# seung-lab/crackle

Hardware: AMD Instinct MI355X
Metric: voxels/s encode+decode, 1024x1024x512 uint32; bit-exact .ckl bytes (higher is better)
Workload: dtype u32

## Files before the change

crackle_amd/csrc/ckl_encode.hip:

```cpp
#include "ckl_encoder.hpp"
#include "ckl_decoder.hpp"
#include "ckl_runs.hpp"
#include "ckl_strips.hpp"
#include "ckl_trail.hpp"
#include "ckl_recompress.hpp"
#include "ckl_erode.hpp"

#include <algorithm>
#include <atomic>
#include <chrono>
#include <functional>
#include <memory>
#include <mutex>

namespace ckl {

using namespace dev;

template <typename LABEL>
__global__ void __launch_bounds__(kBlock) k_stats(const LABEL* __restrict__ labels, uint64_t voxels, unsigned long long* __restrict__ out ) {
	__shared__ unsigned long long s_max[kWaves], s_pairs[kWaves];
	unsigned long long mx = 0, pairs = 0;
	const uint64_t stride = static_cast<uint64_t>(gridDim.x) * kBlock;
	for (uint64_t i = static_cast<uint64_t>(blockIdx.x) * kBlock + threadIdx.x; i < voxels; i += stride) {
// ... 667 lines not shown
	const dim3 grid(static_cast<uint32_t>((threads + kBlock - 1) / kBlock), static_cast<uint32_t>(sz));
	if (four) hipLaunchKernelGGL(k_paint_components4, grid, dim3(kBlock), 0, s, planeV, row_words, plane_words, static_cast<uint32_t>(sx), sxy, word_base, rbase, run_cc, comp_off, id_base, out);
	else hipLaunchKernelGGL(k_paint_components, grid, dim3(kBlock), 0, s, planeV, row_words, plane_words, static_cast<uint32_t>(sx), sxy, word_base, rbase, run_cc, comp_off, id_base, out);
}

__global__ void __launch_bounds__(kBlock) k_bitonic_step(uint64_t* __restrict__ a, uint32_t j, uint32_t k, uint32_t n) {
	const uint32_t i = blockIdx.x * kBlock + threadIdx.x;
	if (i >= n) return;
	const uint32_t l = i ^ j;
	if (l > i) {
		const uint64_t x = a[i], y = a[l];
		const bool up = (i & k) == 0;
		if ((x > y) == up) { a[i] = y; a[l] = x; }
	}
}
__global__ void __launch_bounds__(kBlock) k_bitonic_step2(uint64_t* __restrict__ a, uint32_t j, uint32_t k, uint32_t n) {
	const uint32_t t = blockIdx.x * kBlock + threadIdx.x;
	if (t >= n / 4u) return;
	const uint32_t h = j >> 1;
	const uint32_t lb = static_cast<uint32_t>(__ffs(h)) - 1u;
	const uint32_t i = (t & (h - 1u)) | ((t >> lb) << (lb + 2u));
	uint64_t v0 = a[i], v1 = a[i | h], v2 = a[i | j], v3 = a[i | j | h];
	const bool up = (i & k) == 0;
	auto cx = [&](uint64_t& x, uint64_t& y) { if ((x > y) == up) { const uint64_t z = x; x = y; y = z; } };
	cx(v0, v2); cx(v1, v3);
	cx(v0, v1); cx(v2, v3);
	a[i] = v0; a[i | h] = v1; a[i | j] = v2; a[i | j | h] = v3;
}

__global__ void __launch_bounds__(kBlock) k_bitonic_first(uint64_t* __restrict__ a, uint32_t n) {
	__shared__ uint64_t s[2048];
	const uint32_t base = blockIdx.x * 2048u;
	for (uint32_t t = threadIdx.x; t < 2048u; t += kBlock) s[t] = base + t < n ? a[base + t] : ~0ull;
	__syncthreads();
	for (uint32_t k = 2; k <= 2048u; k <<= 1) {
		for (uint32_t j = k >> 1; j > 0; j >>= 1) {
			for (uint32_t t = threadIdx.x; t < 2048u; t += kBlock) {
				const uint32_t l = t ^ j;
				if (l > t) {
					const uint64_t x = s[t], y = s[l];
					const bool up = ((base + t) & k) == 0;
					if ((x > y) == up) { s[t] = y; s[l] = x; }
				}
			}
			__syncthreads();
		}
	}
	for (uint32_t t = threadIdx.x; t < 2048u; t += kBlock) if (base + t < n) a[base + t] = s[t];
}
__global__ void __launch_bounds__(kBlock) k_bitonic_local(uint64_t* __restrict__ a, uint32_t j_start, uint32_t k, uint32_t n) {
	__shared__ uint64_t s[2048];
	const uint32_t base = blockIdx.x * 2048u;
	for (uint32_t t = threadIdx.x; t < 2048u; t += kBlock) s[t] = base + t < n ? a[base + t] : ~0ull;
	__syncthreads();
	for (uint32_t j = j_start; j > 0; j >>= 1) {
		for (uint32_t t = threadIdx.x; t < 2048u; t += kBlock) {
			const uint32_t l = t ^ j;
			if (l > t) {
				const uint64_t x = s[t], y = s[l];
				const bool up = ((base + t) & k) == 0;
				if ((x > y) == up) { s[t] = y; s[l] = x; }
			}
		}
		__syncthreads();
	}
	for (uint32_t t = threadIdx.x; t < 2048u; t += kBlock) if (base + t < n) a[base + t] = s[t];
}
__global__ void __launch_bounds__(kBlock) k_pad_copy_u64(const uint64_t* __restrict__ src, uint64_t n, uint64_t* __restrict__ dst, uint64_t n_pad) {
	const uint64_t i = static_cast<uint64_t>(blockIdx.x) * kBlock + threadIdx.x;
	if (i < n_pad) dst[i] = i < n ? src[i] : ~0ull;
}
constexpr uint32_t kUniqPer = 8, kUniqItems = kBlock * kUniqPer;
__device__ __forceinline__ uint32_t unique_heads(const uint64_t* __restrict__ sorted, uint32_t n, uint32_t i0, uint64_t (&v)[kUniqPer]) {
	uint32_t flag = 0;
#pragma unroll
	for (uint32_t q = 0; q < kUniqPer; q++) {
		const uint32_t i = i0 + q;
		v[q] = i < n ? sorted[i] : 0;
		const uint64_t prev = q ? v[q - 1] : ((i > 0 && i < n) ? sorted[i - 1] : 0);
		flag |= ((i < n && (i == 0 || v[q] != prev)) ? 1u : 0u) << q;
	}
	return flag;
}
__global__ void __launch_bounds__(kBlock) k_unique_count(const uint64_t* __restrict__ sorted, uint32_t n, uint32_t* __restrict__ blk_count) {
	__shared__ uint32_t s_red[kWaves];
	uint64_t v[kUniqPer];
	const uint32_t flag = unique_heads(sorted, n, blockIdx.x * kUniqItems + threadIdx.x * kUniqPer, v);
	const uint32_t tot = block_sum(static_cast<uint32_t>(__popc(flag)), s_red);
	if (threadIdx.x == 0) blk_count[blockIdx.x] = tot;
}
__global__ void __launch_bounds__(kBlock) k_unique_scan(uint32_t* __restrict__ blk_count, uint32_t nblk, uint32_t* __restrict__ n_uniq) {
	__shared__ uint32_t s_scan[kWaves];
	uint32_t carry = 0;
	for (uint32_t b0 = 0; b0 < nblk; b0 += kBlock) {
		const uint32_t b = b0 + threadIdx.x;
		uint32_t c[1] = { b < nblk ? blk_count[b] : 0u }, tot[1];
		block_excl_add<1>(c, tot, s_scan);
		if (b < nblk) blk_count[b] = carry + c[0];
		carry += tot[0];
	}
	if (threadIdx.x == 0) *n_uniq = carry;
}
__global__ void __launch_bounds__(kBlock) k_unique_scatter(const uint64_t* __restrict__ sorted, uint32_t n, const uint32_t* __restrict__ blk_base, uint64_t* __restrict__ uniq) {
	__shared__ uint32_t s_scan[kWaves];
	uint64_t v[kUniqPer];
	const uint32_t flag = unique_heads(sorted, n, blockIdx.x * kUniqItems + threadIdx.x * kUniqPer, v);
	uint32_t c[1] = { static_cast<uint32_t>(__popc(flag)) }, tot[1];
	block_excl_add<1>(c, tot, s_scan);
	uint32_t o = blk_base[blockIdx.x] + c[0];
#pragma unroll
	for (uint32_t q = 0; q < kUniqPer; q++) if ((flag >> q) & 1u) uniq[o++] = v[q];
}

constexpr uint64_t kLabelHashEmpty = ~0ull;
__device__ __forceinline__ uint32_t label_hash(uint64_t v) {
	v ^= v >> 33; v *= 0xff51afd7ed558ccdull; v ^= v >> 33;
	return static_cast<uint32_t>(v);
}
__global__ void __launch_bounds__(kBlock) k_label_hash_insert(const uint64_t* __restrict__ mapping, uint32_t n, unsigned long long* __restrict__ table, uint32_t mask, uint32_t* __restrict__ has_max) {
	const uint32_t i = blockIdx.x * kBlock + threadIdx.x;
	if (i >= n) return;
	const unsigned long long v = mapping[i];
	if (v == kLabelHashEmpty) { *has_max = 1u; return; }
	uint32_t h = label_hash(v) & mask;
	for (uint32_t probe = 0; probe <= mask; probe++) {
		const unsigned long long seen = table[h];
		if (seen == v) return;
		if (seen == kLabelHashEmpty) {
			const unsigned long long old = atomicCAS(table + h, kLabelHashEmpty, v);
			if (old == kLabelHashEmpty || old == v) return;
		}
		h = (h + 1u) & mask;
	}
}
__device__ __forceinline__ uint32_t hash_occupied(const unsigned long long* __restrict__ table, uint32_t slots, uint32_t i0, uint64_t (&v)[kUniqPer]) {
	uint32_t flag = 0;
#pragma unroll
	for (uint32_t q = 0; q < kUniqPer; q++) {
		v[q] = i0 + q < slots ? table[i0 + q] : kLabelHashEmpty;
		flag |= (v[q] != kLabelHashEmpty ? 1u : 0u) << q;
	}
	return flag;
}
__global__ void __launch_bounds__(kBlock) k_label_hash_count(const unsigned long long* __restrict__ table, uint32_t slots, uint32_t* __restrict__ blk_count) {
	__shared__ uint32_t s_red[kWaves];
	uint64_t v[kUniqPer];
	const uint32_t flag = hash_occupied(table, slots, blockIdx.x * kUniqItems + threadIdx.x * kUniqPer, v);
	const uint32_t tot = block_sum(static_cast<uint32_t>(__popc(flag)), s_red);
	if (threadIdx.x == 0) blk_count[blockIdx.x] = tot;
}
__global__ void __launch_bounds__(kBlock) k_label_hash_scatter(
	const unsigned long long* __restrict__ table, uint32_t slots, const uint32_t* __restrict__ blk_base, const uint32_t* __restrict__ n_found,
	const uint32_t* __restrict__ has_max, uint64_t* __restrict__ out
) {
	__shared__ uint32_t s_scan[kWaves];
	uint64_t v[kUniqPer];
	const uint32_t flag = hash_occupied(table, slots, blockIdx.x * kUniqItems + threadIdx.x * kUniqPer, v);
	uint32_t c[1] = { static_cast<uint32_t>(__popc(flag)) }, tot[1];
	block_excl_add<1>(c, tot, s_scan);
	uint32_t o = blk_base[blockIdx.x] + c[0];
#pragma unroll
	for (uint32_t q = 0; q < kUniqPer; q++) if ((flag >> q) & 1u) out[o++] = v[q];
	if (blockIdx.x == 0 && threadIdx.x == 0 && *has_max) out[*n_found] = kLabelHashEmpty;
}

__global__ void __launch_bounds__(kBlock) k_flat_section(
	const uint64_t* __restrict__ uniq, const uint32_t* __restrict__ n_uniq, int stored_width,
	const uint32_t* __restrict__ ncomp, uint32_t nslices, int component_width,
	const uint64_t* __restrict__ mapping, uint32_t n, uint8_t* __restrict__ out, uint32_t* __restrict__ missing
) {
	const uint32_t nu = *n_uniq;
	const int key_width = nu <= 0xFFu ? 1 : (nu <= 0xFFFFu ? 2 : 4);
	const uint32_t i = blockIdx.x * kBlock + threadIdx.x;
	if (i == 0) for (int b = 0; b < 8; b++) out[b] = static_cast<uint8_t>((static_cast<uint64_t>(nu) >> (8 * b)) & 0xFF);
	uint8_t* o_uniq = out + 8;
	uint8_t* o_cc = o_uniq + static_cast<uint64_t>(nu) * stored_width;
	uint8_t* o_keys = o_cc + static_cast<uint64_t>(nslices) * component_width;
	if (i < nu) {
		const uint64_t v = uniq[i];
		for (int b = 0; b < stored_width; b++) o_uniq[static_cast<uint64_t>(i) * stored_width + b] = static_cast<uint8_t>((v >> (8 * b)) & 0xFF);
	}
	if (i < nslices) {
		const uint32_t v = ncomp[i];
		for (int b = 0; b < component_width; b++) o_cc[static_cast<uint64_t>(i) * component_width + b] = b < 4 ? static_cast<uint8_t>((v >> (8 * b)) & 0xFF) : 0;
	}
	if (i < n) {
		const uint64_t v = mapping[i];
		uint32_t lo = 0, hi = nu;
		while (lo + 1 < hi) {
			const uint32_t mid = (lo + hi) >> 1;
			if (uniq[mid] <= v) lo = mid; else hi = mid;
		}
		if (missing && (nu == 0 || uniq[lo] != v)) *missing = 1u;
		for (int b = 0; b < key_width; b++) o_keys[static_cast<uint64_t>(i) * key_width + b] = static_cast<uint8_t>((lo >> (8 * b)) & 0xFF);
	}
}

__global__ void __launch_bounds__(kBlock) k_code_offsets(
	const uint32_t* __restrict__ boc_len, const uint32_t* __restrict__ payload_len, const uint32_t* __restrict__ slice_err,
	uint32_t nslices, uint64_t* __restrict__ out_off, uint32_t* __restrict__ report
) {
	__shared__ unsigned long long s_part[kBlock];
	__shared__ uint32_t s_err;
	if (threadIdx.x == 0) s_err = 0;
	const uint32_t per = (nslices + kBlock - 1) / kBlock;
	const uint32_t z0 = threadIdx.x * per, z1 = min(z0 + per, nslices);
	unsigned long long sum = 0;
	uint32_t err = 0;
	for (uint32_t z = z0; z < z1; z++) { sum += static_cast<unsigned long long>(boc_len[z]) + payload_len[z]; err |= slice_err[z]; }
	s_part[threadIdx.x] = sum;
	__syncthreads();
	if (err) atomicOr(&s_err, err);
	if (threadIdx.x == 0) {
		unsigned long long run = 0;
		for (uint32_t i = 0; i < kBlock; i++) { const unsigned long long v = s_part[i]; s_part[i] = run; run += v; }
		report[nslices] = static_cast<uint32_t>(run); report[nslices + 1] = static_cast<uint32_t>(run >> 32);
	}
	__syncthreads();
	unsigned long long off = s_part[threadIdx.x];
	for (uint32_t z = z0; z < z1; z++) {
		const uint32_t len = boc_len[z] + payload_len[z];
		out_off[z] = off;
		report[z] = len;
		off += len;
	}
	if (threadIdx.x == 0) report[nslices + 2] = s_err;
}

__global__ void __launch_bounds__(kBlock) k_gather_codes(
	const uint8_t* __restrict__ boc, const uint64_t* __restrict__ bbase, const uint32_t* __restrict__ boc_len,
	const uint8_t* __restrict__ payload, const uint64_t* __restrict__ pbase, const uint32_t* __restrict__ payload_len,
	const uint64_t* __restrict__ out_off, uint8_t* __restrict__ out
) {
	const uint32_t zi = blockIdx.x;
	uint8_t* o = out + out_off[zi];
	const uint32_t nb = boc_len[zi], np = payload_len[zi];
	const uint8_t* b = boc + bbase[zi];
	const uint8_t* p = payload + pbase[zi];
	for (uint32_t i = threadIdx.x; i < nb; i += kBlock) o[i] = b[i];
	for (uint32_t i = threadIdx.x; i < np; i += kBlock) o[nb + i] = p[i];
}

struct CrcShifts { uint32_t x[8]; };
__global__ void __launch_bounds__(kBlock) k_crc32c_pieces(const uint8_t* __restrict__ data, uint64_t n, uint64_t pad, uint32_t P, CrcShifts sh, uint32_t* __restrict__ parts) {
	__shared__ uint32_t s_tab[256];
	__shared__ uint32_t s_st[kBlock];
	{
		uint32_t c = threadIdx.x;
		for (int k = 0; k < 8; k++) c = (c & 1u) ? (c >> 1) ^ dev::kCrcPoly : (c >> 1);
		s_tab[threadIdx.x] = c;
	}
	__syncthreads();
	const uint64_t f0 = (static_cast<uint64_t>(blockIdx.x) * kBlock + threadIdx.x) * P;
	uint32_t c = 0;
	for (uint32_t g = 0; g < P; g += 16) {
		const int64_t m0 = static_cast<int64_t>(f0 + g) - static_cast<int64_t>(pad);
		uint32_t w[4] = { 0, 0, 0, 0 };
		if (m0 >= 0 && static_cast<uint64_t>(m0) + 16u <= n) __builtin_memcpy(w, data + m0, 16);
		else if (m0 + 16 > 0) for (int b = 0; b < 16; b++) { const int64_t i = m0 + b; if (i >= 0 && static_cast<uint64_t>(i) < n) w[b >> 2] |= static_cast<uint32_t>(data[i]) << (8 * (b & 3)); }
#pragma unroll
		for (int b = 0; b < 16; b++) c = s_tab[(c ^ (w[b >> 2] >> (8 * (b & 3)))) & 0xFFu] ^ (c >> 8);
	}
	s_st[threadIdx.x] = c;
	__syncthreads();
	for (int k = 0; k < 8; k++) {
		const uint32_t stride = 1u << k;
		if ((threadIdx.x & (2u * stride - 1u)) == 0u) s_st[threadIdx.x] = gf_mul(s_st[threadIdx.x], sh.x[k]) ^ s_st[threadIdx.x + stride];
		__syncthreads();
	}
	if (threadIdx.x == 0) parts[blockIdx.x] = s_st[0];
}
__global__ void __launch_bounds__(kBlock) k_crc32c_fold(const uint32_t* __restrict__ parts, uint32_t G, CrcShifts sh, uint32_t init_term, uint32_t* __restrict__ out) {
	__shared__ uint32_t s_st[kBlock];
	s_st[threadIdx.x] = threadIdx.x < G ? parts[threadIdx.x] : 0u;
	__syncthreads();
	for (int k = 0; (1u << k) < G; k++) {
		const uint32_t stride = 1u << k;
		if ((threadIdx.x & (2u * stride - 1u)) == 0u && threadIdx.x + stride < G) s_st[threadIdx.x] = gf_mul(s_st[threadIdx.x], sh.x[k]) ^ s_st[threadIdx.x + stride];
		__syncthreads();
	}
	if (threadIdx.x == 0) out[0] = ~(s_st[0] ^ init_term);
}

__global__ void __launch_bounds__(kBlock) k_copy_bytes(const uint8_t* __restrict__ src, uint8_t* __restrict__ dst, uint64_t n) {
	const uint64_t head = min(n, static_cast<uint64_t>((4u - (reinterpret_cast<uintptr_t>(dst) & 3u)) & 3u));
	const uint64_t words = (n - head) / 4u;
	const uint64_t tid = static_cast<uint64_t>(blockIdx.x) * kBlock + threadIdx.x;
	const uint64_t stride = static_cast<uint64_t>(gridDim.x) * kBlock;
	if (tid < head) dst[tid] = src[tid];
	const uint64_t tail0 = head + words * 4u;
	if (tid < n - tail0) dst[tail0 + tid] = src[tail0 + tid];
	const uint8_t* s0 = src + head;
	const uint32_t sh = static_cast<uint32_t>(reinterpret_cast<uintptr_t>(s0) & 3u) * 8u;
	const uint32_t* sw = reinterpret_cast<const uint32_t*>(reinterpret_cast<uintptr_t>(s0) & ~static_cast<uintptr_t>(3));
	uint32_t* dw = reinterpret_cast<uint32_t*>(dst + head);
	if (sh == 0u) {
		for (uint64_t i = tid; i < words; i += stride) dw[i] = sw[i];
	}
	else {
		for (uint64_t i = tid; i < words; i += stride) dw[i] = __funnelshift_r(sw[i], sw[i + 1], sh);
	}
}

__global__ void __launch_bounds__(kBlock) k_trail_step_kinds(const uint32_t* __restrict__ events, const uint64_t* __restrict__ ibase, const uint32_t* __restrict__ n_events, uint32_t* __restrict__ counts) {
	__shared__ uint32_t s_c[5];
	const uint32_t zi = blockIdx.x;
	if (threadIdx.x < 5) s_c[threadIdx.x] = 0u;
	__syncthreads();
	const uint32_t n = n_events[zi] & ~(dev::kEvFormatAddr12 | dev::kEvWalkWide);
	const uint32_t* ev = events + ibase[zi];
	uint32_t c[4] = { 0, 0, 0, 0 };
	for (uint32_t i = threadIdx.x; i < n; i += kBlock) c[ev[i] >> 30]++;
	for (int k = 0; k < 4; k++) if (c[k]) atomicAdd(&s_c[k], c[k]);
	if (threadIdx.x == 0) {
		uint32_t run = 0, longest = 0;
		for (uint32_t i = 0; i < n; i++) { if ((ev[i] >> 30) == 1u) run = 0; else { run++; longest = run > longest ? run : longest; } }
		s_c[4] = longest;
	}
	__syncthreads();
	if (threadIdx.x < 5) counts[zi * 5u + threadIdx.x] = s_c[threadIdx.x];
}

}

using namespace ckl;

static void crc32c_device(const uint8_t* data, uint64_t n, uint32_t* parts, uint32_t* out, hipStream_t s) {
	uint32_t P = 128, G = 1;
	while (G < static_cast<uint32_t>(kBlock) && static_cast<uint64_t>(G) * kBlock * P < n) G <<= 1;
	if (static_cast<uint64_t>(G) * kBlock * P < n) P = static_cast<uint32_t>(((n + static_cast<uint64_t>(G) * kBlock - 1) / (static_cast<uint64_t>(G) * kBlock) + 15) / 16 * 16);
	const uint64_t frame = static_cast<uint64_t>(G) * kBlock * P;
	static std::mutex shifts_mutex;
	static uint32_t shifts_for = 0;
	static CrcShifts shifts_in, shifts_over;
	CrcShifts in_wg, over_wg;
	{
		std::lock_guard<std::mutex> lock(shifts_mutex);
		if (shifts_for != P) {
			for (int k = 0; k < 8; k++) {
				shifts_in.x[k] = gf_xpow(8ull * P << k);
				shifts_over.x[k] = gf_xpow(8ull * P * kBlock << k);
			}
			shifts_for = P;
		}
		in_wg = shifts_in; over_wg = shifts_over;
	}
	hipLaunchKernelGGL(k_crc32c_pieces, dim3(G), dim3(kBlock), 0, s, data, n, frame - n, P, in_wg, parts);
	hipLaunchKernelGGL(k_crc32c_fold, dim3(1), dim3(kBlock), 0, s, parts, G, over_wg, gf_mul(0xFFFFFFFFu, gf_xpow(8ull * n)), out);
}

static void copy_bytes_device(const uint8_t* src, uint8_t* dst, uint64_t n, hipStream_t s) {
	if (!n) return;
	const uint32_t blocks = static_cast<uint32_t>(std::min<uint64_t>((n / 4u + kBlock - 1) / kBlock + 1u, 8192u));
	hipLaunchKernelGGL(k_copy_bytes, dim3(blocks), dim3(kBlock), 0, s, src, dst, n);
}

namespace {

struct UploadPacker {
	struct Item { void* buf; size_t off, count; void (*bind)(void*, uint8_t*, size_t); };
	std::vector<Item> items;
	std::vector<uint8_t> image;
	template <typename T>
	void add(DevBuf<T>& dst, const std::vector<T>& src) {
		const size_t off = (image.size() + 255) & ~static_cast<size_t>(255);
		image.resize(off + std::max<size_t>(src.size(), 1) * sizeof(T));
		if (!src.empty()) memcpy(image.data() + off, src.data(), src.size() * sizeof(T));
		items.push_back({ &dst, off, src.size(), [](void* b, uint8_t* base, size_t n) { static_cast<DevBuf<T>*>(b)->borrow(reinterpret_cast<T*>(base), n); } });
	}
	void commit(DevBuf<uint8_t>& block, hipStream_t s, void** staging = nullptr) {
		if (image.empty()) return;
		for (const Item& it : items) it.bind(it.buf, nullptr, 0);
		block.ensure(image.size());
		if (staging) {
			if (*staging) host_out_free(*staging);
			*staging = host_out_alloc(std::max<size_t>(image.size(), 64u << 10));
			memcpy(*staging, image.data(), image.size());
			upload_small(block.p, *staging, image.size(), s, *staging);
		}
		else CKL_HIP(hipMemcpyAsync(block.p, image.data(), image.size(), hipMemcpyHostToDevice, s));
		for (const Item& it : items) it.bind(it.buf, block.p + it.off, it.count);
	}
};

template <typename LABEL>
VolumeStats volume_stats(ckl_encoder& e, const LABEL* labels, uint64_t voxels) {
	VolumeStats st;
	if (voxels == 0) return st;
	hipStream_t s = e.stream;
	e.d_stats.ensure(2);
	CKL_HIP(hipMemsetAsync(e.d_stats.p, 0, 2 * sizeof(unsigned long long), s));
	const uint32_t blocks = static_cast<uint32_t>(std::min<uint64_t>((voxels + kBlock - 1) / kBlock, 256ull * 8));
	hipLaunchKernelGGL(k_stats<LABEL>, dim3(blocks), dim3(kBlock), 0, s, labels, voxels, e.d_stats.p);
	auto r = download(e.d_stats.p, 2, s);
	st.max_label = r[0]; st.pairs = r[1];
	LABEL f, l;
	CKL_HIP(hipMemcpy(&f, labels, sizeof(LABEL), hipMemcpyDeviceToHost));
	CKL_HIP(hipMemcpy(&l, labels + (voxels - 1), sizeof(LABEL), hipMemcpyDeviceToHost));
	st.first = f; st.last = l;
	return st;
}

inline uint32_t* plane_v(const ckl_encoder& e) { return e.d_planes.p; }
inline uint32_t* plane_h(const ckl_encoder& e, uint32_t ns) { return e.d_planes.p + e.plane_words * ns; }

inline bool planes_cached(const ckl_encoder& e, const void* labels, int64_t sx, int64_t sy, int64_t sz) {
	return e.planes_for == labels && e.planes_dims[0] == sx && e.planes_dims[1] == sy && e.planes_dims[2] == sz;
}

inline uint64_t crack_edges(const ckl_encoder& e, int64_t sx, int64_t sy, size_t zi, bool permissible) {
	const uint64_t interior = static_cast<uint64_t>(sx > 0 ? sx - 1 : 0) * sy + static_cast<uint64_t>(sx) * (sy > 0 ? sy - 1 : 0);
	const uint64_t differ = static_cast<uint64_t>(e.count_v[zi]) + e.count_h[zi];
	return permissible ? interior - differ : differ;
}

void planes_collect(ckl_encoder& e, uint32_t ns, VolumeStats* st, const std::vector<unsigned long long>* fetched = nullptr) {
	std::vector<unsigned long long> mine;
	if (!fetched) { mine = download(e.d_plane_out.p, 4ull * ns, e.stream); fetched = &mine; }
	const std::vector<unsigned long long>& o = *fetched;
	e.count_v.resize(ns); e.count_h.resize(ns);
	VolumeStats v;
	for (uint32_t zi = 0; zi < ns; zi++) {
		e.count_v[zi] = static_cast<uint32_t>(o[4ull * zi]);
		e.count_h[zi] = static_cast<uint32_t>(o[4ull * zi + 1]);
		v.pairs += o[4ull * zi + 2];
		v.max_label = std::max<uint64_t>(v.max_label, o[4ull * zi + 3]);
	}
	e.planes_deferred = false;
	if (st) *st = v;
}

void trail_prezero(ckl_encoder& e, int64_t sx, int64_t sy, int64_t sz) {
	hipStream_t s = e.stream2;
	const uint32_t ns = static_cast<uint32_t>(sz);
	const uint64_t nverts = static_cast<uint64_t>(sx + 1) * (sy + 1);
	const uint32_t start_words = static_cast<uint32_t>((nverts + 31) / 32);
	e.d_slice_err.ensure(ns);
	e.t_counters.ensure(7 * static_cast<size_t>(ns));
	e.t_start_bits.ensure(static_cast<size_t>(start_words) * ns);
	CKL_HIP(hipMemsetAsync(e.d_slice_err.p, 0, ns * sizeof(uint32_t), s));
	CKL_HIP(hipMemsetAsync(e.t_counters.p, 0, 7 * static_cast<size_t>(ns) * sizeof(uint32_t), s));
	CKL_HIP(hipMemsetAsync(e.t_start_bits.p, 0, static_cast<size_t>(start_words) * ns * sizeof(uint32_t), s));
	CKL_HIP(hipEventRecord(e.ev_prezero, s));
	e.trail_zeroed = true;
}

template <typename LABEL>
void planes_pass(ckl_encoder& e, const LABEL* labels, int64_t sx, int64_t sy, int64_t sz, VolumeStats* st, bool defer = false) {
	hipStream_t s = e.stream;
	const uint32_t ns = static_cast<uint32_t>(sz);
	e.trail_zeroed = false;
	e.planes_deferred = false;
	e.row_words = static_cast<uint32_t>((sx + 31) / 32);
	e.plane_words = static_cast<uint64_t>(e.row_words) * sy;
	e.d_planes.ensure(2 * e.plane_words * ns);
	constexpr uint32_t P = 16 / sizeof(LABEL);
	const bool fast = !getenv("CKL_PLANES_GENERIC") && sx >= static_cast<int64_t>(P) && sx % P == 0 && (reinterpret_cast<uintptr_t>(labels) & 15u) == 0;
	if (fast) {
		const uint32_t strips = static_cast<uint32_t>((sx + 64 * P - 1) / (64 * P));
		const uint32_t bands = static_cast<uint32_t>((sy + kBandRows - 1) / kBandRows);
		const uint32_t nblk = (strips * bands + kWaves - 1) / kWaves;
		e.d_plane_partial.ensure(4ull * nblk * ns);
		e.d_plane_partial_max.ensure(static_cast<size_t>(nblk) * ns);
		e.d_plane_out.ensure(4ull * ns + 1);
		trail_prezero(e, sx, sy, sz);
		hipLaunchKernelGGL(k_label_planes_stream<LABEL>, dim3(nblk, ns), dim3(kBlock), 0, s,
			labels, static_cast<uint32_t>(sx), static_cast<uint32_t>(sy), strips, bands,
			plane_v(e), plane_h(e, ns), e.row_words, e.plane_words,
			e.d_plane_partial.p, e.d_plane_partial_max.p, e.d_plane_out.p + 4ull * ns);
		hipLaunchKernelGGL(k_planes_reduce, dim3(ns), dim3(kBlock), 0, s, e.d_plane_partial.p, e.d_plane_partial_max.p, nblk, e.d_plane_out.p, e.d_plane_out.p + 4ull * ns);
		e.planes_deferred = defer;
		if (!e.planes_deferred) planes_collect(e, ns, st);
		return;
	}
	if (st) *st = volume_stats<LABEL>(e, labels, static_cast<uint64_t>(sx) * sy * sz);
	e.d_count_vh.ensure(2 * static_cast<size_t>(ns));
	CKL_HIP(hipMemsetAsync(e.d_count_vh.p, 0, 2 * static_cast<size_t>(ns) * sizeof(uint32_t), s));
	const uint32_t chunks = static_cast<uint32_t>((sx + 63) / 64);
	const uint64_t units = static_cast<uint64_t>(chunks) * sy;
	hipLaunchKernelGGL(k_label_planes<LABEL>, dim3(static_cast<uint32_t>((units + kWaves * kPlaneUnroll - 1) / (kWaves * kPlaneUnroll)), ns), dim3(kBlock), 0, s,
		labels, static_cast<uint32_t>(sx), static_cast<uint32_t>(sy), chunks,
		plane_v(e), plane_h(e, ns), e.row_words, e.plane_words,
		e.d_count_vh.p, e.d_count_vh.p + ns);
	std::vector<uint32_t> c = download(e.d_count_vh.p, 2 * static_cast<size_t>(ns), s);
	e.count_v.assign(c.begin(), c.begin() + ns);
	e.count_h.assign(c.begin() + ns, c.end());
}

void planes_pass_any(ckl_encoder& e, const void* labels, int64_t sx, int64_t sy, int64_t sz, VolumeStats* st) {
	with_label_type(e.dtype_bytes, [&](auto t) { planes_pass(e, static_cast<const typename decltype(t)::type*>(labels), sx, sy, sz, st); });
}

enum class GraphFormat : uint32_t { IMPERMISSIBLE = 0, PERMISSIBLE = 1, ON_DEVICE = 2 };
inline GraphFormat graph_format(bool permissible) { return permissible ? GraphFormat::PERMISSIBLE : GraphFormat::IMPERMISSIBLE; }
void graph_pass(ckl_encoder& e, int64_t sx, int64_t sy, int64_t sz, GraphFormat format, VolumeStats* st = nullptr) {
	hipStream_t s = e.stream;
	const uint32_t ns = static_cast<uint32_t>(sz);
	e.tiles_x = static_cast<uint32_t>((sx + 1 + kTrailTileDim - 1) / kTrailTileDim);
	e.tiles_y = static_cast<uint32_t>((sy + 1 + 7) / 8);
	const uint32_t mtx = static_cast<uint32_t>((sx + 1 + 7) / 8), mty = static_cast<uint32_t>((sy + 1 + 7) / 8);
	e.mtx2 = (mtx + 1) / 2;
	e.adjm_stride = static_cast<uint64_t>(e.mtx2) * ((mty + 1) / 2) * 4 * 2;
	e.d_adjm.ensure(e.adjm_stride * ns);
	e.graph_blocks = (e.tiles_x * e.tiles_y + kBlock - 1) / kBlock;
	e.t_blk_special.ensure(static_cast<size_t>(e.graph_blocks) * ns);
	e.t_blk_corner.ensure(static_cast<size_t>(e.graph_blocks) * ns);
	e.d_count_vh.ensure(4 * static_cast<size_t>(ns));
	const bool on_device = format == GraphFormat::ON_DEVICE;
	if (on_device && !e.planes_deferred) throw Error(CKL_ERR_RUNTIME, "crackle_amd: internal: crack format left to the device without deferred counts");
	const unsigned long long half_voxels = static_cast<unsigned long long>(static_cast<int64_t>(static_cast<uint64_t>(sx) * sy * sz) / 2);
	hipLaunchKernelGGL(k_trail_graph, dim3(e.graph_blocks, ns), dim3(kBlock), 0, s,
		plane_v(e), plane_h(e, ns), e.row_words, e.plane_words,
		static_cast<uint32_t>(sx), static_cast<uint32_t>(sy), static_cast<uint32_t>(format),
		on_device ? e.d_plane_out.p + 4ull * ns : nullptr, half_voxels,
		reinterpret_cast<uint32_t*>(e.d_adjm.p), e.adjm_stride * 4,
		e.mtx2, e.tiles_x, e.tiles_y, e.t_blk_special.p, e.t_blk_corner.p);
	hipLaunchKernelGGL(k_trail_count_scan, dim3(ns), dim3(kBlock), 0, s, e.t_blk_special.p, e.t_blk_corner.p, e.graph_blocks,
		e.d_count_vh.p + 2 * static_cast<size_t>(ns), e.d_count_vh.p + 3 * static_cast<size_t>(ns));
	std::vector<unsigned long long> po;
	if (e.planes_deferred) {
		po.resize(4ull * ns);
		CKL_HIP(hipMemcpyAsync(po.data(), e.d_plane_out.p, po.size() * sizeof(unsigned long long), hipMemcpyDeviceToHost, s));
	}
	std::vector<uint32_t> c = download(e.d_count_vh.p + 2 * static_cast<size_t>(ns), 2 * static_cast<size_t>(ns), s);
	e.count_special.assign(c.begin(), c.begin() + ns);
	e.count_corner.assign(c.begin() + ns, c.end());
	VolumeStats v;
	if (!po.empty()) planes_collect(e, ns, &v, &po);
	if (st && !po.empty()) *st = v;
	e.graph_permissible = on_device ? static_cast<int64_t>(v.pairs) < static_cast<int64_t>(static_cast<uint64_t>(sx) * sy * sz) / 2 : format == GraphFormat::PERMISSIBLE;
}

enum class CrackGoal { HISTOGRAM, CODES };
struct CrackRequest {
	CrackGoal goal = CrackGoal::CODES;
	bool permissible = false;
	int markov_order = 0;
	const std::vector<uint8_t>* model = nullptr;
	bool reuse_trail = false;
	std::function<void()> overlap;
};
struct CrackResult {
	std::vector<uint32_t> code_len;
	uint64_t total = 0;
	bool any_chain = false;
	std::vector<uint32_t> hist;
	std::vector<uint8_t> model;
};

inline size_t trail_walk_lds(uint32_t max_special) { return (static_cast<size_t>(max_special) + 256) * 16 + 1024; }

FinishArgs finish_args(const ckl_encoder& e, int64_t sx, int64_t sy, int markov_order) {
	FinishArgs fa;
	fa.sx = static_cast<int>(sx); fa.sy = static_cast<int>(sy);
	fa.xw = byte_width(static_cast<uint64_t>(sx) + 1); fa.yw = byte_width(static_cast<uint64_t>(sy) + 1);
	fa.markov = markov_order ? 1u : 0u;
	fa.cbase = e.d_cbase.p; fa.kbase = e.d_kbase.p;
	fa.n_chains = e.d_n_chains.p; fa.n_raw = e.d_n_raw.p; fa.n_valid = e.d_n_valid.p;
	fa.cp = e.d_cp.p; fa.chain_node = e.d_chain_node.p; fa.chain_off = e.d_chain_off.p; fa.chain_clen = e.d_chain_clen.p;
	fa.chain_order = e.d_chain_order.p; fa.chain_dst = e.d_chain_dst.p; fa.chain_vstart = e.d_chain_vstart.p;
	fa.fcode = e.d_fcode.p; fa.dcode = e.d_dcode.p;
	fa.pbase = e.d_pbase.p; fa.payload = e.d_payload.p; fa.bbase = e.d_bbase.p; fa.boc = e.d_boc.p;
	fa.payload_len = e.d_payload_len.p; fa.boc_len = e.d_boc_len.p;
	fa.z0 = 0;
	return fa;
}

TrailArgs trail_args(const ckl_encoder& e, int64_t sx, int64_t sy, uint32_t ns) {
	const uint64_t nverts = static_cast<uint64_t>(sx + 1) * (sy + 1);
	TrailArgs ta;
	ta.adjm = e.d_adjm.p; ta.adjm_stride = e.adjm_stride; ta.mtx2 = e.mtx2; ta.tiles_x = e.tiles_x; ta.tiles_y = e.tiles_y;
	ta.planeV = plane_v(e); ta.planeH = plane_h(e, ns); ta.row_words = e.row_words; ta.plane_words = e.plane_words;
	ta.sx = static_cast<uint32_t>(sx); ta.sy = static_cast<uint32_t>(sy); ta.inv = e.graph_permissible ? 0xFFFFFFFFu : 0u;
	ta.sxe = static_cast<uint32_t>(sx + 1); ta.sye = static_cast<uint32_t>(sy + 1); ta.nverts = static_cast<uint32_t>(nverts);
	ta.max_steps = e.t_max_steps.p;
	ta.nbase = e.t_nbase.p; ta.ncap = e.t_ncap.p;
	ta.n_nodes = e.t_counters.p; ta.n_corners = e.t_counters.p + 2 * ns;
	ta.n_starts = e.t_counters.p + 3 * ns; ta.n_items = e.t_counters.p + 4 * ns;
	ta.node_vertex = e.t_node_vertex.p; ta.node_adj = e.t_node_adj.p; ta.vert2node = e.t_vert2node.p;
	ta.cobase = e.t_cobase.p; ta.cocap = e.t_cocap.p; ta.corner_vertex = e.t_corner_vertex.p;
	ta.dart_end = e.t_dart_end.p; ta.dart_len = e.t_dart_len.p; ta.dart_minv = e.t_dart_minv.p; ta.dart_minpos = e.t_dart_minpos.p;
	ta.dart_codes = e.t_dart_codes.p; ta.dart_inline = e.t_dart_inline.p;
	ta.parent = e.t_parent.p; ta.compmin = e.t_compmin.p;
	ta.start_bits = e.t_start_bits.p; ta.start_words = static_cast<uint32_t>((nverts + 31) / 32); ta.starts = e.t_starts.p;
	ta.ibase = e.t_ibase.p; ta.icap = e.t_icap.p; ta.items = e.t_items.p; ta.item_off = e.t_item_off.p;
	ta.sbase = e.d_sbase.p; ta.scap = e.d_scap.p; ta.stack_node = e.d_stack_node.p; ta.stack_item = e.d_stack_code.p;
	ta.kbase = e.d_kbase.p; ta.kcap = e.d_kcap.p;
	ta.chain_node = e.d_chain_node.p; ta.chain_item0 = e.t_chain_item0.p; ta.chain_off = e.d_chain_off.p; ta.chain_clen = e.d_chain_clen.p;
	ta.n_chains = e.d_n_chains.p; ta.n_raw = e.d_n_raw.p; ta.n_valid = e.d_n_valid.p;
	ta.cbase = e.d_cbase.p; ta.ccap = e.d_ccap.p; ta.cp = e.d_cp.p; ta.slice_err = e.d_slice_err.p;
	ta.events = e.t_events.p; ta.n_events = e.t_counters.p + 5 * ns; ta.seg_len_sum = e.t_counters.p + 6 * ns; ta.chain_ev0 = e.t_chain_ev0.p; ta.ev_lnd = e.t_ev_lnd.p; ta.ev_item = e.t_ev_item.p;
	ta.dbg = nullptr;
	{ const char* env = getenv("CKL_TRAIL_WALK"); ta.walk_plain = (env && !strcmp(env, "plain")) ? 1u : 0u; ta.walk_no_regs = (env && !strcmp(env, "lds")) ? 1u : 0u; }
	{ const char* env = getenv("CKL_TRAIL_WALK_STACK"); ta.walk_stack_cap = env ? static_cast<uint32_t>(std::max(1, atoi(env))) : 0xFFFFFFFFu; }
	ta.graph_blocks = e.graph_blocks; ta.blk_special = e.t_blk_special.p; ta.blk_corner = e.t_blk_corner.p;
	ta.z0 = 0;
	return ta;
}

void trail_diag(ckl_encoder& e, uint32_t ns, const unsigned long long* ta_dbg, uint32_t max_special, size_t trail_lds_used) {
	hipStream_t s = e.stream;
	std::vector<uint32_t> c = download(e.t_counters.p, 5 * static_cast<size_t>(ns), s);
	double m[5] = { 0 };
	for (int k = 0; k < 5; k++) for (uint32_t zi = 0; zi < ns; zi++) m[k] += static_cast<double>(c[static_cast<size_t>(k) * ns + zi]) / ns;
	double sp = 0, co = 0;
	for (uint32_t zi = 0; zi < ns; zi++) { sp += static_cast<double>(e.count_special[zi]) / ns; co += static_cast<double>(e.count_corner[zi]) / ns; }
	if (ta_dbg) {
		std::vector<unsigned long long> g = download(ta_dbg, 16, s);
		if (g[11]) fprintf(stderr, "[ckl trail diag, k_trail_walk] mean cycles per slice: table fill=%.0f fill + walk=%.0f\n", static_cast<double>(g[6]) / g[11], static_cast<double>(g[7]) / g[11]);
		if (g[11]) fprintf(stderr, "[ckl trail diag, k_trail_walk] slices=%llu iterations/slice=%.0f cycles/iteration=%.0f clock=%.2f GHz (cycles / 100 MHz ticks)\n",
			g[11], static_cast<double>(g[8]) / g[11], g[8] ? static_cast<double>(g[9]) / g[8] : 0.0, g[10] ? static_cast<double>(g[9]) / (g[10] * 10.0) : 0.0);
		fprintf(stderr, "[ckl trail diag, k_trail_components, mean cycles per slice] union=%.0f component minima=%.0f starts/splits=%.0f bitmap scan=%.0f\n",
			static_cast<double>(g[12]) / ns, static_cast<double>(g[13]) / ns, static_cast<double>(g[14]) / ns, static_cast<double>(g[15]) / ns);
		fprintf(stderr, "[ckl trail diag, k_trail_segments] waves=%llu iterations/wave mean=%.1f max=%llu cycles/wave mean=%.0f max=%llu cycles/iteration=%.0f active lanes/iteration=%.1f\n",
			g[4], g[4] ? static_cast<double>(g[0]) / g[4] : 0.0, g[1], g[4] ? static_cast<double>(g[2]) / g[4] : 0.0, g[3],
			g[0] ? static_cast<double>(g[2]) / g[0] : 0.0, g[0] ? static_cast<double>(g[5]) / g[0] : 0.0);
	}
	fprintf(stderr, "[ckl trail diag] max degree-1/3/4 vertices of a slice=%u, k_trail_walk LDS=%zu bytes\n", max_special, trail_lds_used);
	fprintf(stderr, "[ckl trail diag, mean per slice] degree-1/3/4 vertices=%.0f corners=%.0f nodes=%.0f starts=%.0f items=%.0f\n", sp, co, m[0], m[3], m[4]);
}

void check_walk_errors(ckl_encoder& e, uint32_t ns) {
	const std::vector<uint32_t> errs = download(e.d_slice_err.p, ns, e.stream);
	for (uint32_t zi = 0; zi < ns; zi++) if (errs[zi]) throw Error(CKL_ERR_RUNTIME, "crackle_amd: crack walk scratch overflow on z=" + std::to_string(zi));
}

CrackResult crack_pass(ckl_encoder& e, int64_t sx, int64_t sy, int64_t sz, const CrackRequest& rq) {
	hipStream_t s = e.stream;
	const uint32_t ns = static_cast<uint32_t>(sz);
	const uint64_t nverts = static_cast<uint64_t>(sx + 1) * (sy + 1);
	const int markov_order = rq.markov_order;
	const bool reuse_trail = rq.reuse_trail;
	if (rq.goal == CrackGoal::HISTOGRAM && (!markov_order || rq.model)) throw Error(CKL_ERR_RUNTIME, "crackle_amd: internal: a markov histogram needs an order and no model");
	CrackResult result;
	e.d_slice_err.ensure(ns);
	const bool prezeroed = e.trail_zeroed && !reuse_trail;
	e.trail_zeroed = false;
	if (prezeroed) CKL_HIP(hipStreamWaitEvent(s, e.ev_prezero, 0));
	if (!reuse_trail && !prezeroed) CKL_HIP(hipMemsetAsync(e.d_slice_err.p, 0, ns * sizeof(uint32_t), s));

	std::vector<uint64_t> cbase(ns), sbase(ns), kbase(ns);
	std::vector<uint32_t> ccap(ns), scap(ns), kcap(ns), max_steps(ns);
	std::vector<uint64_t> nbase(ns), cobase(ns), ibase(ns);
	std::vector<uint32_t> ncap(ns), cocap(ns), icap(ns);
	uint64_t ctot = 0, stot = 0, ktot = 0, ntot = 0, cotot = 0, itot = 0;
	uint32_t max_ncap = 0, max_cocap = 0, max_icap = 0, max_special = 0;
	bool any = false;
	for (uint32_t zi = 0; zi < ns; zi++) {
		const uint64_t E = crack_edges(e, sx, sy, zi, rq.permissible);
		any = any || E > 0;
		const uint64_t cc = ((7 * E + 16 + 15) / 16) * 16;
		if (cc > 0xFFFFFFF0ull) throw Error(CKL_ERR_RUNTIME, "crackle_amd: slice has too many crack edges");
		cbase[zi] = ctot; ccap[zi] = static_cast<uint32_t>(cc); ctot += cc;
		max_steps[zi] = static_cast<uint32_t>(E + 1);
		const uint64_t nc = ((static_cast<uint64_t>(e.count_special[zi]) + e.count_corner[zi] + 16) / 16) * 16;
		if (nc >= (1ull << 28)) throw Error(CKL_ERR_RUNTIME, "crackle_amd: slice has too many crack vertices");
		nbase[zi] = ntot; ncap[zi] = static_cast<uint32_t>(nc); ntot += nc;
		cobase[zi] = cotot; cocap[zi] = e.count_corner[zi]; cotot += e.count_corner[zi];
		const uint64_t ic = 7 * nc + 16;
		ibase[zi] = itot; icap[zi] = static_cast<uint32_t>(ic); itot += ic;
		sbase[zi] = stot; scap[zi] = static_cast<uint32_t>(2 * nc + 4); stot += 2 * nc + 4;
		kbase[zi] = ktot; kcap[zi] = static_cast<uint32_t>(nc); ktot += nc;
		max_ncap = std::max<uint32_t>(max_ncap, ncap[zi]);
		max_cocap = std::max<uint32_t>(max_cocap, cocap[zi]);
		max_icap = std::max<uint32_t>(max_icap, icap[zi]);
		max_special = std::max<uint32_t>(max_special, e.count_special[zi]);
	}
	result.any_chain = any;
	if (g_ht && g_ht->on) {
		uint32_t over = 0;
		for (uint32_t zi = 0; zi < ns; zi++) over += e.count_special[zi] > 3584u;
		fprintf(stderr, "[ckl trail nodes] max special %u, slices above 3584: %u of %u\n", max_special, over, ns);
	}
	HT_MARK("c:caps");

	UploadPacker tables;
	tables.add(e.d_cbase, cbase); tables.add(e.d_ccap, ccap);
	tables.add(e.d_sbase, sbase); tables.add(e.d_scap, scap);
	tables.add(e.d_kbase, kbase); tables.add(e.d_kcap, kcap);
	e.d_cp.ensure(ctot); e.d_fcode.ensure(ctot);
	if (markov_order) e.d_dcode.ensure(ctot);
	e.d_stack_node.ensure(stot); e.d_stack_code.ensure(stot);
	e.d_chain_node.ensure(ktot); e.d_chain_off.ensure(ktot); e.d_chain_clen.ensure(ktot);
	e.d_chain_order.ensure(ktot); e.d_chain_dst.ensure(ktot); e.d_chain_vstart.ensure(ktot);
	e.d_n_chains.ensure(ns); e.d_n_raw.ensure(ns); e.d_n_valid.ensure(ns);
	e.d_payload_len.ensure(ns); e.d_boc_len.ensure(ns);
	const int xw = byte_width(static_cast<uint64_t>(sx) + 1), yw = byte_width(static_cast<uint64_t>(sy) + 1);
	std::vector<uint64_t> pbase(ns), bbase(ns);
	uint64_t ptot = 0, btot = 0;
	for (uint32_t zi = 0; zi < ns; zi++) {
		const uint64_t ncodes = ccap[zi];
		const uint64_t pbytes = markov_order ? (3ull * ncodes + 2 + 7) / 8 : (ncodes + 3) / 4;
		pbase[zi] = ptot; ptot += ((pbytes + 8 + 3) / 4) * 4;
		const uint64_t bbytes = 4 + yw + static_cast<uint64_t>(kcap[zi]) * (yw + 2 * xw);
		bbase[zi] = btot; btot += bbytes;
	}
	tables.add(e.d_pbase, pbase); tables.add(e.d_bbase, bbase);
	tables.add(e.t_nbase, nbase); tables.add(e.t_ncap, ncap);
	tables.add(e.t_cobase, cobase); tables.add(e.t_cocap, cocap);
	tables.add(e.t_ibase, ibase); tables.add(e.t_icap, icap);
	tables.add(e.t_max_steps, max_steps);
	tables.commit(e.d_crack_tables, s, e.uploads_by_kernel ? &e.tables_staging : nullptr);
	HT_MARK("c:tables");
	e.d_payload.ensure(ptot + 8); e.d_boc.ensure(btot + 8);
	e.codes_capacity = ptot + btot;
	if (markov_order) CKL_HIP(hipMemsetAsync(e.d_payload.p, 0, ptot + 8, s));

	DevBuf<unsigned long long> d_tdbg;
	size_t trail_lds_used = 0;
	if (!reuse_trail) {
		e.t_counters.ensure(7 * static_cast<size_t>(ns));
		if (!prezeroed) CKL_HIP(hipMemsetAsync(e.t_counters.p, 0, 7 * static_cast<size_t>(ns) * sizeof(uint32_t), s));
		e.t_node_vertex.ensure(ntot); e.t_node_adj.ensure(ntot + 16); e.t_vert2node.ensure(nverts * ns);
		e.t_corner_vertex.ensure(cotot);
		e.t_dart_end.ensure(4 * ntot); e.t_dart_len.ensure(4 * ntot); e.t_dart_minv.ensure(4 * ntot); e.t_dart_minpos.ensure(4 * ntot);
		e.t_dart_codes.ensure(4 * ntot); e.t_dart_inline.ensure(4 * ntot);
		e.t_parent.ensure(ntot); e.t_compmin.ensure(ntot); e.t_starts.ensure(ntot);
		const uint32_t start_words = static_cast<uint32_t>((nverts + 31) / 32);
		e.t_start_bits.ensure(static_cast<size_t>(start_words) * ns);
		if (!prezeroed) CKL_HIP(hipMemsetAsync(e.t_start_bits.p, 0, static_cast<size_t>(start_words) * ns * sizeof(uint32_t), s));
		e.t_items.ensure(itot); e.t_item_off.ensure(itot); e.t_chain_item0.ensure(ktot);
		e.t_events.ensure(itot); e.t_chain_ev0.ensure(ktot); e.t_ev_lnd.ensure(itot); e.t_ev_item.ensure(itot);
		e.last_trail_slices = ns;

		TrailArgs ta = trail_args(e, sx, sy, ns);
		const FinishArgs fa = finish_args(e, sx, sy, markov_order);
		if (kTuning && getenv("CKL_TRAIL_DIAG")) { d_tdbg.ensure(16); CKL_HIP(hipMemsetAsync(d_tdbg.p, 0, 128, s)); ta.dbg = d_tdbg.p; }
		int max_lds = 0;
		CKL_HIP(hipDeviceGetAttribute(&max_lds, hipDeviceAttributeMaxSharedMemoryPerBlock, e.device));
		const size_t budget = static_cast<size_t>(max_lds > 1024 ? max_lds - 1024 : 0);
		const uint32_t dart_blocks = (4 * max_ncap + kWalkChunk * kWaves - 1) / (kWalkChunk * kWaves);
		size_t clds = (static_cast<size_t>(max_special) + 1024) * 12;
		if (const char* env = getenv("CKL_TRAIL_LDS")) clds = static_cast<size_t>(std::max(0, atoi(env)));
		clds = (std::min(budget, std::max<size_t>(clds, 1024)) / 16) * 16;
		CKL_HIP(hipFuncSetAttribute(reinterpret_cast<const void*>(&k_trail_components), hipFuncAttributeMaxDynamicSharedMemorySize, static_cast<int>(clds)));
		size_t lds = trail_walk_lds(max_special);
		if (const char* env = getenv("CKL_TRAIL_LDS")) lds = static_cast<size_t>(std::max(0, atoi(env)));
		lds = std::min(budget, std::max<size_t>(lds, 4096));
		lds = (lds / 16) * 16;
		CKL_HIP(hipFuncSetAttribute(reinterpret_cast<const void*>(&k_trail_walk), hipFuncAttributeMaxDynamicSharedMemorySize, static_cast<int>(lds)));
		trail_lds_used = lds;
		HT_MARK("c:setup");

		if (any) {
			hipLaunchKernelGGL(k_trail_nodes, dim3(e.graph_blocks, ns), dim3(kBlock), 0, s, ta);
			hipLaunchKernelGGL(k_trail_segments, dim3(dart_blocks, ns), dim3(kBlock), 0, s, ta);
			if (max_cocap) hipLaunchKernelGGL(k_trail_loops, dim3((max_cocap + kBlock - 1) / kBlock, ns), dim3(kBlock), 0, s, ta);
			hipLaunchKernelGGL(k_trail_components, dim3(ns), dim3(kCompBlock), clds, s, ta, static_cast<uint32_t>(clds));
		}
		CKL_HIP(hipEventRecord(e.evd0, s));
		hipLaunchKernelGGL(k_trail_walk, dim3(ns), dim3(kWave), lds, s, ta, static_cast<uint32_t>(lds));
		CKL_HIP(hipEventRecord(e.evd1, s));
		hipLaunchKernelGGL(k_trail_items, dim3(ns), dim3(kItemsBlock), 0, s, ta);
		hipLaunchKernelGGL(k_trail_offsets, dim3(ns), dim3(kBlock), 0, s, ta);
		hipLaunchKernelGGL(k_trail_expand, dim3((max_icap + kExpandChunk * kWaves - 1) / (kExpandChunk * kWaves), ns), dim3(kBlock), 0, s, ta);
		hipLaunchKernelGGL(k_finish, dim3(ns), dim3(kFinishBlock), 0, s, fa);
	}
	HT_MARK("c:enqueue");
	if (kTuning && getenv("CKL_TRAIL_DIAG")) trail_diag(e, ns, d_tdbg.p, max_special, trail_lds_used);

	auto enqueue_tail = [&]() {
		e.d_out_off.ensure(ns);
		e.d_code_report.ensure(static_cast<size_t>(ns) + 3);
		e.d_codes_out.ensure(e.codes_capacity + 8);
		hipLaunchKernelGGL(k_code_offsets, dim3(1), dim3(kBlock), 0, s, e.d_boc_len.p, e.d_payload_len.p, e.d_slice_err.p, ns, e.d_out_off.p, e.d_code_report.p);
		hipLaunchKernelGGL(k_gather_codes, dim3(ns), dim3(kBlock), 0, s, e.d_boc.p, e.d_bbase.p, e.d_boc_len.p,
			e.d_payload.p, e.d_pbase.p, e.d_payload_len.p, e.d_out_off.p, e.d_codes_out.p);
	};
	if (!markov_order) enqueue_tail();
	if (rq.overlap) rq.overlap();
	HT_MARK("c:overlap");

	if (markov_order) {
		if (rq.model) result.model = *rq.model;
		else {
			const size_t rows = static_cast<size_t>(1) << (2 * markov_order);
			e.d_hist.ensure(rows * 4);
			CKL_HIP(hipMemsetAsync(e.d_hist.p, 0, rows * 4 * sizeof(uint32_t), s));
			const uint32_t hist_lds = (rows * 4 <= 16384) ? static_cast<uint32_t>(rows * 4) : 0u;
			if (hist_lds * 4 > 48 * 1024) CKL_HIP(hipFuncSetAttribute(reinterpret_cast<const void*>(&k_markov_hist), hipFuncAttributeMaxDynamicSharedMemorySize, static_cast<int>(hist_lds * 4)));
			hipLaunchKernelGGL(k_markov_hist, dim3(ns), dim3(kBlock), hist_lds * sizeof(uint32_t), s, e.d_dcode.p, e.d_cbase.p, e.d_n_valid.p, markov_order, e.d_hist.p, hist_lds);
			result.hist = download(e.d_hist.p, rows * 4, s);
			if (rq.goal == CrackGoal::HISTOGRAM) { check_walk_errors(e, ns); return result; }
			result.model = markov_stats_to_model(result.hist.data(), rows);
		}
		upload(e.d_model, result.model, s);
		hipLaunchKernelGGL(k_markov_pack, dim3(ns), dim3(kBlock), 0, s, e.d_dcode.p, e.d_cbase.p, e.d_n_valid.p, markov_order,
			e.d_model.p, e.d_pbase.p, e.d_payload.p, e.d_payload_len.p);
		enqueue_tail();
	}
	HT_MARK("c:finish_enq");
	const std::vector<uint32_t> report = download(e.d_code_report.p, static_cast<size_t>(ns) + 3, s);
	HT_MARK("c:finish_wait");
	if (report[ns + 2]) check_walk_errors(e, ns);
	result.code_len.assign(report.begin(), report.begin() + ns);
	result.total = static_cast<uint64_t>(report[ns]) | (static_cast<uint64_t>(report[ns + 1]) << 32);
	return result;
}

struct FlatResult {
	std::vector<uint32_t> ncomp;
	std::vector<uint32_t> crcs;
	uint64_t total = 0;
};

void ensure_geom_table(ckl_encoder& e, uint64_t sxy) {
	if (e.g_table_pixels == sxy && e.d_G.p) return;
	hipStream_t s = e.stream2;
	const uint32_t npx = static_cast<uint32_t>(sxy);
	const uint32_t B = 1024, nblk = npx / B + 1;
	std::vector<uint32_t> g_base(B), blk_g(nblk), blk_x(nblk);
	const uint32_t X = gf_xpow(32);
	g_base[0] = 0;
	for (uint32_t i = 1; i < B; i++) g_base[i] = gf_mul(X, g_base[i - 1] ^ 0x80000000u);
	const uint32_t gB = gf_mul(X, g_base[B - 1] ^ 0x80000000u);
	const uint32_t XB = gf_xpow(32ull * B);
	blk_g[0] = 0; blk_x[0] = 0x80000000u;
	for (uint32_t k = 1; k < nblk; k++) {
		blk_g[k] = blk_g[k - 1] ^ gf_mul(blk_x[k - 1], gB);
		blk_x[k] = gf_mul(blk_x[k - 1], XB);
	}
	DevBuf<uint32_t> t_base, t_g, t_x;
	upload(t_base, g_base, s); upload(t_g, blk_g, s); upload(t_x, blk_x, s);
	e.d_G.ensure(static_cast<size_t>(npx) + 1);
	hipLaunchKernelGGL(k_build_geom_table, dim3(npx / kBlock + 1), dim3(kBlock), 0, s, t_base.p, t_g.p, t_x.p, npx, e.d_G.p);
	CKL_HIP(hipStreamSynchronize(s));
	e.g_table_pixels = sxy;
}

RunArrays flat_arrays(const ckl_encoder& e) {
	RunArrays ra;
	ra.word_base = e.d_word_base.p; ra.rbase = e.d_rbase.p; ra.rcap = e.d_rcap.p;
	ra.parent = e.d_parent.p; ra.run_start = e.d_run_start.p; ra.run_cc = e.d_run_cc.p;
	ra.nruns = e.d_nruns.p; ra.ncomp = e.d_ncomp.p; ra.slice_err = e.d_slice_err2.p;
	ra.comp_pix = e.d_comp_pix.p;
	return ra;
}

void flat_report_layout(ckl_encoder& e, uint32_t ns, hipStream_t s) {
	e.d_flat_report.ensure(4 * static_cast<size_t>(ns) + 1);
	e.d_ncomp.borrow(e.d_flat_report.p, ns); e.d_crc_acc.borrow(e.d_flat_report.p + ns, ns);
	e.d_idbits.borrow(e.d_flat_report.p + 2 * static_cast<size_t>(ns), ns); e.d_slice_err2.borrow(e.d_flat_report.p + 3 * static_cast<size_t>(ns), ns);
	CKL_HIP(hipMemsetAsync(e.d_slice_err2.p, 0, (static_cast<size_t>(ns) + 1) * sizeof(uint32_t), s));
}

RunGeom flat_geom(const ckl_encoder& e, int64_t sx, int64_t sy, uint32_t ns) {
	RunGeom g;
	g.planeV = plane_v(e); g.planeH = plane_h(e, ns);
	g.row_words = e.row_words; g.plane_words = e.plane_words;
	g.flip = 1u;
	g.sx = static_cast<uint32_t>(sx); g.sy = static_cast<uint32_t>(sy);
	return g;
}

void flat_enqueue_runs(ckl_encoder& e, int64_t sx, int64_t sy, int64_t sz) {
	hipStream_t s = e.stream2;
	const uint32_t ns = static_cast<uint32_t>(sz);
	const uint64_t sxy = static_cast<uint64_t>(sx) * sy;
	e.flat_strips = false;

	std::vector<uint64_t>& rbase = e.h_rbase;
	std::vector<uint32_t>& rcap = e.h_rcap;
	rbase.assign(ns, 0); rcap.assign(ns, 0);
	uint64_t rtot = 0;
	uint32_t max_rcap = 0;
	for (uint32_t zi = 0; zi < ns; zi++) {
		const uint64_t runs = static_cast<uint64_t>(sy) + e.count_v[zi];
		rbase[zi] = rtot; rcap[zi] = static_cast<uint32_t>(runs); rtot += runs;
		max_rcap = std::max<uint32_t>(max_rcap, static_cast<uint32_t>(runs));
	}
	upload(e.d_rbase, rbase, s); upload(e.d_rcap, rcap, s);
	e.d_word_base.ensure(e.plane_words * ns);
	e.d_parent.ensure(rtot); e.d_run_start.ensure(rtot); e.d_run_cc.ensure(rtot); e.d_comp_pix.ensure(rtot);
	e.d_nruns.ensure(ns);
	flat_report_layout(e, ns, s);

	const RunGeom g = flat_geom(e, sx, sy, ns);
	const RunArrays ra = flat_arrays(e);
	hipLaunchKernelGGL(k_run_index, dim3(ns), dim3(kIndexBlock), 0, s, g, ra);
	launch_run_union(s, ns, g, ra);
	ResolveScratch rs;
	rs.nblk = (max_rcap + kBlock - 1) / kBlock;
	e.d_run_local.ensure(rtot);
	e.d_blk_roots.ensure(static_cast<size_t>(rs.nblk) * ns);
	rs.run_local = e.d_run_local.p; rs.blk_roots = e.d_blk_roots.p;
	launch_run_resolve(s, ns, ra, rs, e.d_G.p, static_cast<uint32_t>(sxy), 0u, e.d_crc_acc.p, e.d_idbits.p);
	HT_MARK("f:enqueue_runs");
}

uint32_t flat_resolve_cap(size_t lds_bytes) {
	uint32_t cap = static_cast<uint32_t>(std::min<size_t>(kResolveCap, (lds_bytes - (kMaxStrips + 64u) * 4u) / 4u));
	if (const char* env = getenv("CKL_ENC_RESOLVE_CAP")) cap = std::min<uint32_t>(cap, static_cast<uint32_t>(std::max(1, atoi(env))));
	return cap;
}
uint32_t flat_resolve_cap_max(ckl_encoder& e) {
	if (!e.max_lds) CKL_HIP(hipDeviceGetAttribute(&e.max_lds, hipDeviceAttributeMaxSharedMemoryPerBlock, e.device));
	return flat_resolve_cap(static_cast<size_t>(e.max_lds) - 8192u);
}

bool flat_strip_plan(ckl_encoder& e, int64_t sx, int64_t sy, uint32_t ns) {
	if (getenv("CKL_ENC_LABEL_RUNS")) return false;
	const uint64_t sxy = static_cast<uint64_t>(sx) * sy;
	if (e.row_words == 0 || e.row_words > kStripWords || sxy >= 0xFFFF0000ull) return false;
	uint64_t runs_max = 0, comps_min = 0;
	const uint64_t pairs_up = static_cast<uint64_t>(sx) * (sy - 1);
	for (uint32_t zi = 0; zi < ns; zi++) {
		const uint64_t runs = static_cast<uint64_t>(sy) + e.count_v[zi];
		const uint64_t equal_up = pairs_up - std::min<uint64_t>(pairs_up, e.count_h[zi]);
		runs_max = std::max<uint64_t>(runs_max, runs);
		comps_min = std::max<uint64_t>(comps_min, runs > equal_up ? runs - equal_up : 0ull);
	}
	const double runs_per_row = static_cast<double>(runs_max) / static_cast<double>(sy);
	const uint32_t fit = static_cast<uint32_t>(0.7 * kEncStripCap / runs_per_row);
	if (fit < 1u) return false;
	const uint32_t rows = std::max<uint32_t>(1u, std::min<uint32_t>(kStripWords / e.row_words, fit));
	const uint32_t nstrips = (static_cast<uint32_t>(sy) + rows - 1) / rows;
	if (nstrips > kMaxStrips || comps_min > flat_resolve_cap_max(e)) return false;
	e.flat_strip_rows = rows; e.flat_nstrips = nstrips;
	e.flat_strip_cap = static_cast<uint32_t>(std::min<uint64_t>(kEncStripCap, static_cast<uint64_t>(rows) * sx));
	if (const char* env = getenv("CKL_ENC_STRIP_CAP")) e.flat_strip_cap = std::min<uint32_t>(e.flat_strip_cap, static_cast<uint32_t>(std::max(1, atoi(env))));
	return true;
}

StripArrays flat_strip_arrays(const ckl_encoder& e) {
	StripArrays sa = {};
	sa.run_lid = e.s_run_lid.p; sa.sc_w = e.s_sc_w.p; sa.sc_cc = e.s_sc_first.p;
	sa.strip_nruns = e.s_strip_nruns.p; sa.strip_nsc = e.s_strip_nsc.p;
	sa.seam_first = e.s_seam_first.p; sa.seam_last = e.s_seam_last.p;
	sa.slice_err = e.d_slice_err2.p; sa.overflow = e.d_flat_report.p + 4 * e.d_ncomp.n;
	sa.nstrips = e.flat_nstrips; sa.strip_rows = e.flat_strip_rows; sa.cap = e.flat_strip_cap; sa.zbase = 0;
	return sa;
}

void flat_launch_resolve(ckl_encoder& e, const void* labels, int64_t sx, int64_t sy, uint32_t ns, uint32_t cap) {
	hipStream_t s = e.stream2;
	e.flat_resolve_cap = cap;
	e.d_label_slots.ensure(static_cast<size_t>(ns) * cap);
	ResolveArgs ra = {};
	ra.cap = cap;
	EncResolve en;
	en.labels = labels; en.sxy = static_cast<uint64_t>(sx) * sy; en.slots = e.d_label_slots.p; en.crc_acc = e.d_crc_acc.p; en.idbits = e.d_idbits.p;
	const RunGeom g = flat_geom(e, sx, sy, ns);
	const StripArrays sa = flat_strip_arrays(e);
	const size_t tab_bytes = static_cast<size_t>(cap) * sizeof(uint32_t);
	if (e.label_src) {
		if (tab_bytes > 48u * 1024u) CKL_HIP(hipFuncSetAttribute(reinterpret_cast<const void*>(&k_slice_resolve_enc_pixels), hipFuncAttributeMaxDynamicSharedMemorySize, static_cast<int>(tab_bytes)));
		hipLaunchKernelGGL(k_slice_resolve_enc_pixels, dim3(ns), dim3(kResolveBlock), tab_bytes, s, g, sa, ra, en, e.d_ncomp.p);
		return;
	}
	with_label_type(e.dtype_bytes, [&](auto t) {
		typedef typename decltype(t)::type LABEL;
		if (tab_bytes > 48u * 1024u) CKL_HIP(hipFuncSetAttribute(reinterpret_cast<const void*>(&k_slice_resolve_enc<LABEL>), hipFuncAttributeMaxDynamicSharedMemorySize, static_cast<int>(tab_bytes)));
		hipLaunchKernelGGL(k_slice_resolve_enc<LABEL>, dim3(ns), dim3(kResolveBlock), tab_bytes, s, g, sa, ra, en, e.d_ncomp.p);
	});
}

void flat_enqueue(ckl_encoder& e, const void* labels, int64_t sx, int64_t sy, int64_t sz, bool need_runs, bool beside_walk) {
	hipStream_t s = e.stream2;
	const uint32_t ns = static_cast<uint32_t>(sz);
	const uint64_t sxy = static_cast<uint64_t>(sx) * sy;
	ensure_geom_table(e, sxy);
	if (need_runs || !beside_walk || !flat_strip_plan(e, sx, sy, ns)) { flat_enqueue_runs(e, sx, sy, sz); return; }
	e.flat_strips = true;
	const size_t nst = static_cast<size_t>(e.flat_nstrips) * ns;
	e.s_strip_nruns.ensure(nst); e.s_strip_nsc.ensure(nst);
	e.s_seam_first.ensure(nst * e.row_words); e.s_seam_last.ensure(nst * e.row_words);
	e.s_run_lid.ensure(nst * e.flat_strip_cap); e.s_sc_w.ensure(nst * e.flat_strip_cap); e.s_sc_first.ensure(nst * e.flat_strip_cap);
	flat_report_layout(e, ns, s);
	hipLaunchKernelGGL(k_strip_ccl_enc, dim3(e.flat_nstrips, ns), dim3(kBlock), 0, s, flat_geom(e, sx, sy, ns), flat_strip_arrays(e), e.d_G.p, static_cast<uint32_t>(sxy));
	flat_launch_resolve(e, labels, sx, sy, ns, flat_resolve_cap(kFlatResolveLds));
	HT_MARK("f:enqueue_strips");
}

template <typename LABEL>
void flat_collect(ckl_encoder& e, const LABEL* labels, int64_t sx, int64_t sy, int64_t sz, FlatResult& out) {
	hipStream_t s = e.stream2;
	const uint32_t ns = static_cast<uint32_t>(sz);
	const uint64_t sxy = static_cast<uint64_t>(sx) * sy;
	const size_t rep_n = 4 * static_cast<size_t>(ns) + 1;
	std::vector<uint32_t> rep = download(e.d_flat_report.p, rep_n, s);
	if (e.flat_strips && rep[rep_n - 1] == 2u && e.flat_resolve_cap < flat_resolve_cap_max(e)) {
		CKL_HIP(hipMemsetAsync(e.d_flat_report.p + rep_n - 1, 0, sizeof(uint32_t), s));
		flat_launch_resolve(e, labels, sx, sy, ns, flat_resolve_cap_max(e));
		HT_MARK("f:resolve_retry");
		rep = download(e.d_flat_report.p, rep_n, s);
	}
	if (e.flat_strips && rep[rep_n - 1]) {
		flat_enqueue_runs(e, sx, sy, sz);
		rep = download(e.d_flat_report.p, rep_n, s);
	}
	const uint32_t *acc = rep.data() + ns, *idbits = rep.data() + 2 * static_cast<size_t>(ns), *errs = rep.data() + 3 * static_cast<size_t>(ns);
	out.ncomp.assign(rep.begin(), rep.begin() + ns);
	HT_MARK(e.flat_strips ? "f:wait_strips" : "f:wait_runs");
	for (uint32_t zi = 0; zi < ns; zi++) if (errs[zi]) throw Error(CKL_ERR_RUNTIME, "crackle_amd: run table overflow on z=" + std::to_string(zi));
	const uint32_t init_term = gf_mul(0xFFFFFFFFu, gf_xpow(32ull * sxy));
	out.crcs.resize(ns);
	uint32_t fix_bits = 0xFFFFFFFFu, fix = 0;
	for (uint32_t zi = 0; zi < ns; zi++) {
		if (idbits[zi] != fix_bits) { fix_bits = idbits[zi]; fix = gf_xpow(32 - fix_bits); }
		out.crcs[zi] = ~(gf_mul(acc[zi], fix) ^ init_term);
	}

	std::vector<uint64_t>& comp_off = e.h_comp_off;
	comp_off.assign(ns, 0);
	uint64_t total = 0;
	for (uint32_t zi = 0; zi < ns; zi++) { comp_off[zi] = total; total += out.ncomp[zi]; }
	upload(e.d_comp_off, comp_off, s);
	e.d_mapping.ensure(total + 1);
	uint32_t max_ncomp = 1;
	for (uint32_t zi = 0; zi < ns; zi++) max_ncomp = std::max(max_ncomp, out.ncomp[zi]);
	const dim3 grid((max_ncomp + kBlock - 1) / kBlock, ns);
	if (e.label_src) hipLaunchKernelGGL(k_component_labels_from_runs, grid, dim3(kBlock), 0, s, *e.label_src,
		e.flat_strips ? e.d_label_slots.p : nullptr, e.flat_resolve_cap, e.d_comp_pix.p, e.d_rbase.p, e.d_ncomp.p, e.d_comp_off.p, e.d_mapping.p);
	else if (e.flat_strips) hipLaunchKernelGGL(k_gather_slots, grid, dim3(kBlock), 0, s, e.d_label_slots.p, e.flat_resolve_cap, e.d_ncomp.p, e.d_comp_off.p, e.d_mapping.p);
	else hipLaunchKernelGGL(k_mapping_comps<LABEL>, grid, dim3(kBlock), 0, s, labels, flat_arrays(e), sxy, e.d_comp_off.p, e.d_mapping.p);
	out.total = total;
}

uint64_t flat_section(ckl_encoder& e, uint64_t N, int stored_width, int component_width, uint32_t ns, const ckl_encode_overrides* ov = nullptr) {
	hipStream_t s = e.stream2;
	if (N > 0x7FFFFFFFull) throw Error(CKL_ERR_RUNTIME, "crackle_amd: too many components");
	e.d_n_uniq.ensure(2);
	e.d_uniq.ensure(N + 1);
	const uint64_t* sort_src = e.d_mapping.p;
	uint64_t n_sort = N;
	if (N > 8192 && N <= (1ull << 26) && !getenv("CKL_LABEL_SORT_ALL")) {
		uint32_t slots = 16384;
		while (slots < 2 * N) slots <<= 1;
		e.d_label_hash.ensure(slots);
		CKL_HIP(hipMemsetAsync(e.d_label_hash.p, 0xFF, static_cast<size_t>(slots) * sizeof(uint64_t), s));
		CKL_HIP(hipMemsetAsync(e.d_n_uniq.p, 0, 2 * sizeof(uint32_t), s));
		unsigned long long* table = reinterpret_cast<unsigned long long*>(e.d_label_hash.p);
		hipLaunchKernelGGL(k_label_hash_insert, dim3(static_cast<uint32_t>((N + kBlock - 1) / kBlock)), dim3(kBlock), 0, s, e.d_mapping.p, static_cast<uint32_t>(N), table, slots - 1u, e.d_n_uniq.p + 1);
		const uint32_t hb = (slots + kUniqItems - 1) / kUniqItems;
		e.d_uniq_blk.ensure(hb + 1);
		hipLaunchKernelGGL(k_label_hash_count, dim3(hb), dim3(kBlock), 0, s, table, slots, e.d_uniq_blk.p);
		hipLaunchKernelGGL(k_unique_scan, dim3(1), dim3(kBlock), 0, s, e.d_uniq_blk.p, hb, e.d_n_uniq.p);
		hipLaunchKernelGGL(k_label_hash_scatter, dim3(hb), dim3(kBlock), 0, s, table, slots, e.d_uniq_blk.p, e.d_n_uniq.p, e.d_n_uniq.p + 1, e.d_uniq.p);
		const std::vector<uint32_t> found = download(e.d_n_uniq.p, 2, s);
		n_sort = static_cast<uint64_t>(found[0]) + (found[1] ? 1u : 0u);
		if (n_sort == 0 || n_sort > N) throw Error(CKL_ERR_RUNTIME, "crackle_amd: label table pass failed");
		e.d_label_list.ensure(n_sort);
		CKL_HIP(hipMemcpyAsync(e.d_label_list.p, e.d_uniq.p, n_sort * sizeof(uint64_t), hipMemcpyDeviceToDevice, s));
		sort_src = e.d_label_list.p;
	}
	const bool merge_unsorted = ov && ov->merge_unique && sort_src == e.d_label_list.p;
	uint32_t n_pad = 2048;
	while (n_pad < n_sort) n_pad <<= 1;
	if (!merge_unsorted) {
	e.d_sorted.ensure(n_pad);
	const uint32_t blocks = (n_pad + kBlock - 1) / kBlock;
	hipLaunchKernelGGL(k_pad_copy_u64, dim3(blocks), dim3(kBlock), 0, s, sort_src, n_sort, e.d_sorted.p, static_cast<uint64_t>(n_pad));
	hipLaunchKernelGGL(k_bitonic_first, dim3(n_pad / 2048), dim3(kBlock), 0, s, e.d_sorted.p, n_pad);
	for (uint32_t k = 4096; k <= n_pad; k <<= 1) {
		uint32_t j = k >> 1;
		for (; j >= 4096 && !getenv("CKL_BITONIC_SINGLE_STEPS"); j >>= 2) hipLaunchKernelGGL(k_bitonic_step2, dim3((n_pad / 4 + kBlock - 1) / kBlock), dim3(kBlock), 0, s, e.d_sorted.p, j, k, n_pad);
		for (; j >= 2048; j >>= 1) hipLaunchKernelGGL(k_bitonic_step, dim3(blocks), dim3(kBlock), 0, s, e.d_sorted.p, j, k, n_pad);
		hipLaunchKernelGGL(k_bitonic_local, dim3(n_pad / 2048), dim3(kBlock), 0, s, e.d_sorted.p, j, k, n_pad);
	}
	{
		const uint32_t ub = static_cast<uint32_t>((n_sort + kUniqItems - 1) / kUniqItems);
		e.d_uniq_blk.ensure(ub + 1);
		hipLaunchKernelGGL(k_unique_count, dim3(ub), dim3(kBlock), 0, s, e.d_sorted.p, static_cast<uint32_t>(n_sort), e.d_uniq_blk.p);
		hipLaunchKernelGGL(k_unique_scan, dim3(1), dim3(kBlock), 0, s, e.d_uniq_blk.p, ub, e.d_n_uniq.p);
		hipLaunchKernelGGL(k_unique_scatter, dim3(ub), dim3(kBlock), 0, s, e.d_sorted.p, static_cast<uint32_t>(n_sort), e.d_uniq_blk.p, e.d_uniq.p);
	}
	}
	uint64_t uniq_bound = N;
	const bool merged_list = ov && ov->merge_unique;
	if (ov && ov->merge_unique) {
		HT_MARK("l:enqueue");
		const uint32_t n_local = merge_unsorted ? static_cast<uint32_t>(n_sort) : download(e.d_n_uniq.p, 1, s)[0];
		std::vector<uint64_t> local = download(merge_unsorted ? e.d_label_list.p : e.d_uniq.p, n_local, s);
		HT_MARK("l:local");
		const uint64_t* merged = nullptr;
		uint64_t n_merged = 0;
		if (ov->merge_unique(ov->merge_ctx, local.data(), n_local, &merged, &n_merged) != 0 || (!merged && n_merged))
			throw Error(CKL_ERR_RUNTIME, "crackle_amd: the merge_unique callback failed");
		HT_MARK("l:merge");
		if (n_merged < n_local || n_merged > 0xFFFFFFFFull) throw Error(CKL_ERR_ARG, "crackle_amd: merge_unique returned a list that cannot contain the slab's labels");
		e.d_uniq.ensure(n_merged + 1);
		if (n_merged) CKL_HIP(hipMemcpyAsync(e.d_uniq.p, merged, n_merged * sizeof(uint64_t), hipMemcpyHostToDevice, s));
		const uint32_t nm[2] = { static_cast<uint32_t>(n_merged), 0u };
		CKL_HIP(hipMemcpyAsync(e.d_n_uniq.p, nm, sizeof(nm), hipMemcpyHostToDevice, s));
		CKL_HIP(hipStreamSynchronize(s));
		e.d_labels_bin.ensure(8 + n_merged * static_cast<uint64_t>(stored_width) + static_cast<uint64_t>(ns) * component_width + N * 4 + 16);
		uniq_bound = std::max<uint64_t>(uniq_bound, n_merged);
	}
	e.d_labels_bin.ensure(8 + N * static_cast<uint64_t>(stored_width) + static_cast<uint64_t>(ns) * component_width + N * 4 + 16);
	const uint64_t work = std::max<uint64_t>(std::max<uint64_t>(uniq_bound, ns), 1);
	hipLaunchKernelGGL(k_flat_section, dim3(static_cast<uint32_t>((work + kBlock - 1) / kBlock)), dim3(kBlock), 0, s,
		e.d_uniq.p, e.d_n_uniq.p, stored_width, e.d_ncomp.p, ns, component_width, e.d_mapping.p, static_cast<uint32_t>(N), e.d_labels_bin.p,
		merged_list ? e.d_n_uniq.p + 1 : nullptr);
	HT_MARK("l:enqueue");
	const std::vector<uint32_t> report = download(e.d_n_uniq.p, merged_list ? 2 : 1, s);
	const uint32_t nu = report[0];
	HT_MARK("l:wait");
	if (merged_list && report[1]) throw Error(CKL_ERR_ARG, "crackle_amd: merge_unique returned a list that lacks a label of the slab");
	return 8 + static_cast<uint64_t>(nu) * stored_width + static_cast<uint64_t>(ns) * component_width + N * static_cast<uint64_t>(byte_width(nu));
}

Header stream_header(int data_width, int64_t sx, int64_t sy, int64_t sz, const VolumeStats& st, bool allow_pins, bool fortran_order, uint64_t markov_model_order, const ckl_encode_overrides* ov) {
	Header head;
	head.crack_format = IMPERMISSIBLE;
	head.label_format = PINS_VARIABLE_WIDTH;
	if (static_cast<int64_t>(st.pairs) < static_cast<int64_t>(static_cast<uint64_t>(sx) * sy * sz) / 2) {
		head.crack_format = PERMISSIBLE;
		head.label_format = FLAT;
	}
	if (ov && ov->force_crack_format >= 0) {
		head.crack_format = ov->force_crack_format;
		head.label_format = ov->force_crack_format == PERMISSIBLE ? FLAT : PINS_VARIABLE_WIDTH;
	}
	if (sz == 1 || !allow_pins) head.label_format = FLAT;
	if (ov && ov->force_label_format >= 0) head.label_format = ov->force_label_format;
	head.is_signed = false;
	head.data_width = data_width;
	head.stored_data_width = ov && ov->force_stored_width ? ov->force_stored_width : byte_width(st.max_label);
	head.sx = static_cast<uint32_t>(sx); head.sy = static_cast<uint32_t>(sy); head.sz = static_cast<uint32_t>(sz);
	head.log2_grid_size = 31;
	head.fortran_order = fortran_order;
	head.markov_model_order = static_cast<int>(markov_model_order & 0xFF);
	head.is_sorted = true;
	return head;
}
inline std::vector<uint8_t> header_bytes(const Header& head) {
	std::vector<uint8_t> hb;
	head.write(hb);
	return hb;
}

template <typename LABEL>
void encode_typed(
	ckl_encoder& e, const LABEL* labels, int64_t sx, int64_t sy, int64_t sz,
	bool allow_pins, bool fortran_order, uint64_t markov_model_order,
	bool optimize_pins, bool auto_bgcolor, int64_t manual_bgcolor,
	const ckl_encode_overrides* ov, uint8_t** out, uint64_t* out_len
) {
	const uint64_t voxels = static_cast<uint64_t>(sx) * sy * sz;
	hipStream_t s = e.stream;
	CKL_HIP(hipEventRecord(e.ev0, s));

	HostTimer ht;
	g_ht = &ht;
	VolumeStats st;
	e.trail_zeroed = false;
	const bool have_planes = voxels > 0 && (e.label_src ? planes_cached(e, e.label_src, sx, sy, sz) : ov && planes_cached(e, labels, sx, sy, sz));
	e.planes_for = nullptr;
	if (e.label_src && voxels > 0 && !have_planes) throw Error(CKL_ERR_RUNTIME, "crackle_amd: internal: recompress without its planes");
	const bool labels_first = getenv("CKL_NO_OVERLAP") || static_cast<uint64_t>(sx) * sy > (1536ull * 1536ull)
		|| (getenv("CKL_LABELS_AT_WALK") && atoi(getenv("CKL_LABELS_AT_WALK")) == 0);
	if (voxels > 0 && !have_planes) planes_pass<LABEL>(e, labels, sx, sy, sz, &st, !labels_first);
	else if (have_planes) st = e.planes_stats;
	ht.mark("planes");
	bool graph_done = false;
	if (e.planes_deferred) {
		e.trail_for = nullptr;
		graph_pass(e, sx, sy, sz, ov && ov->force_crack_format >= 0 ? graph_format(ov->force_crack_format == PERMISSIBLE) : GraphFormat::ON_DEVICE, &st);
		graph_done = true;
		ht.mark("graph");
	}
	Header head = stream_header(static_cast<int>(sizeof(LABEL)), sx, sy, sz, st, allow_pins, fortran_order, markov_model_order, ov);
	const int stored_width = head.stored_data_width;
	e.uploads_by_kernel = head.label_format == FLAT;
	if (voxels == 0) { hand_out(header_bytes(head), OutAlloc::MALLOC, out, out_len); return; }
	if (optimize_pins) throw Error(CKL_ERR_ARG, "crackle_amd: allow_pins=2 (find_optimal_pins) is out of scope");
	if (head.label_format != FLAT && head.label_format != PINS_VARIABLE_WIDTH) throw Error(CKL_ERR_ARG, "crackle_amd: unsupported label format");
	if (head.markov_model_order > 13) throw Error(CKL_ERR_ARG, "crackle_amd: markov_model_order > 13 is not supported on device");

	bool labels_at_walk = false;
	const bool need_runs = head.label_format != FLAT;
	if (labels_first && !graph_done) flat_enqueue(e, labels, sx, sy, sz, need_runs, false);
	const bool trail_cached = !graph_done && have_planes && ov && ov->has_model && head.markov_model_order > 0 && e.trail_for == static_cast<const void*>(labels)
		&& e.trail_perm == (head.crack_format == PERMISSIBLE) && e.trail_order == head.markov_model_order;
	e.trail_for = nullptr;
	if (graph_done && e.graph_permissible != (head.crack_format == PERMISSIBLE)) throw Error(CKL_ERR_RUNTIME, "crackle_amd: internal: device and host disagree on the crack format");
	if (!trail_cached && !graph_done) graph_pass(e, sx, sy, sz, graph_format(head.crack_format == PERMISSIBLE));
	ht.mark("graph");
	if (!labels_first) {
		uint32_t max_special = 0;
		for (uint32_t v : e.count_special) max_special = std::max(max_special, v);
		int max_lds = 0;
		CKL_HIP(hipDeviceGetAttribute(&max_lds, hipDeviceAttributeMaxSharedMemoryPerBlock, e.device));
		labels_at_walk = max_special < 5000 && 2 * trail_walk_lds(max_special) + kFlatResolveLds <= static_cast<size_t>(max_lds);
		if (!labels_at_walk) flat_enqueue(e, labels, sx, sy, sz, need_runs, false);
	}

	const bool permissible = head.crack_format == PERMISSIBLE;
	{
		bool any = false;
		for (int64_t z = 0; z < sz && !any; z++) any = crack_edges(e, sx, sy, z, permissible) > 0;
		if (!any && !(ov && ov->has_model)) head.markov_model_order = 0;
	}
	std::vector<uint8_t> forced_model;
	CrackRequest crq;
	crq.permissible = permissible;
	crq.markov_order = head.markov_model_order;
	crq.reuse_trail = trail_cached;
	if (ov && ov->has_model && head.markov_model_order > 0) {
		const size_t rows = static_cast<size_t>(1) << (2 * head.markov_model_order);
		forced_model.assign(ov->model, ov->model + rows * 4);
		crq.model = &forced_model;
	}

	FlatResult fr;
	std::vector<uint8_t> pins_binary;
	uint64_t label_bytes = 0;
	const uint64_t off_index = Header::kBytes;
	const uint64_t off_labels = off_index + 4ull * (sz + 1);
	uint64_t est_code_bytes = 0;
	{
		const int xw = byte_width(static_cast<uint64_t>(sx) + 1), yw = byte_width(static_cast<uint64_t>(sy) + 1);
		for (int64_t z = 0; z < sz; z++) {
			const uint64_t codes = crack_edges(e, sx, sy, z, permissible) + 4ull * (static_cast<uint64_t>(e.count_special[z]) + e.count_corner[z]) + 16;
			est_code_bytes += (head.markov_model_order ? (3 * codes + 7) / 8 : (codes + 3) / 4) + 8;
			est_code_bytes += 4 + yw + 64ull * (yw + 2 * xw);
		}
	}
	if (getenv("CKL_SMALL_ESTIMATE")) est_code_bytes = 0;
	const uint64_t model_bytes_est = head.markov_model_order ? (1ull << (2 * head.markov_model_order)) : 0;
	struct HostOut { void* p = nullptr; ~HostOut() { if (p) host_out_free(p); } } early;
	uint64_t early_cap = 0;
	uint32_t labels_crc = 0;
	const int component_width = byte_width(static_cast<uint64_t>(sx) * sy);
	hipStream_t s2 = e.stream2;
	bool labels_stay = false;
	auto label_side = [&]() {
		if (labels_at_walk) {
			CKL_HIP(hipStreamWaitEvent(s2, e.evd0, 0));
			flat_enqueue(e, labels, sx, sy, sz, need_runs, true);
		}
		flat_collect<LABEL>(e, labels, sx, sy, sz, fr);
		HT_MARK("flat");
		const uint64_t N = fr.total;
		if (head.label_format == PINS_VARIABLE_WIDTH) {
			if (N > 0xFFFFFFFFull) throw Error(CKL_ERR_RUNTIME, "crackle_amd: too many components");
			e.d_cc_volume.ensure(voxels);
			launch_paint_components(s2, plane_v(e), e.row_words, e.plane_words, sx, sy, sz, e.d_word_base.p, e.d_rbase.p, e.d_run_cc.p, e.d_comp_off.p, 0u, e.d_cc_volume.p);
			pins_binary = pins_section_plain<LABEL>(e, labels, e.d_cc_volume.p, e.d_mapping.p, sx, sy, sz, N, fr.ncomp, head.pin_index_width(), stored_width, auto_bgcolor, manual_bgcolor);
			label_bytes = pins_binary.size();
		}
		else {
			label_bytes = flat_section(e, N, stored_width, component_width, static_cast<uint32_t>(sz), ov);
			HT_MARK("label_table");
			labels_stay = e.async_host_copy && e.keep_device_stream && !e.defer_codes && label_bytes > 0;
			early_cap = off_labels + label_bytes + model_bytes_est + est_code_bytes + 4ull * (sz + 1) + 64;
			early.p = host_out_alloc(early_cap);
			HT_MARK("l:buffer");
			uint8_t* eo = static_cast<uint8_t*>(early.p);
			if (labels_stay) {
				e.d_labels_crc.ensure(1 + kBlock);
				if (!e.ev_labels_crc) CKL_HIP(hipEventCreateWithFlags(&e.ev_labels_crc, hipEventDisableTiming));
				crc32c_device(e.d_labels_bin.p, label_bytes, e.d_labels_crc.p + 1, e.d_labels_crc.p, s2);
				CKL_HIP(hipEventRecord(e.ev_labels_crc, s2));
			}
			else {
				if (label_bytes) CKL_HIP(hipMemcpyAsync(eo + off_labels, e.d_labels_bin.p, label_bytes, hipMemcpyDeviceToHost, s2));
				CKL_HIP(hipStreamSynchronize(s2));
				labels_crc = crc32c(eo + off_labels, label_bytes);
			}
			HT_MARK("labels_d2h");
		}
	};

	const bool no_overlap = getenv("CKL_NO_OVERLAP") != nullptr;
	if (!no_overlap) crq.overlap = label_side;
	const CrackResult cr = crack_pass(e, sx, sy, sz, crq);
	if (no_overlap) label_side();
	ht.mark("cracks");
	std::vector<uint8_t> stored_model;
	if (head.markov_model_order > 0) stored_model = markov_model_to_stored(cr.model);

	head.num_label_bytes = label_bytes;
	const uint64_t off_model = off_labels + label_bytes;
	const uint64_t off_codes = off_model + stored_model.size();
	const uint64_t off_tail = off_codes + cr.total;
	const uint64_t total = off_tail + 4ull * (sz + 1);
	uint8_t* o;
	if (early.p && total <= early_cap) { o = static_cast<uint8_t*>(early.p); early.p = nullptr; }
	else {
		o = static_cast<uint8_t*>(host_out_alloc(total));
		if (early.p && label_bytes) memcpy(o + off_labels, static_cast<uint8_t*>(early.p) + off_labels, label_bytes);
	}
	try {
		e.last_codes_total = cr.total;
		if (head.label_format == PINS_VARIABLE_WIDTH) {
			if (label_bytes) memcpy(o + off_labels, pins_binary.data(), label_bytes);
			labels_crc = crc32c(o + off_labels, label_bytes);
		}
		std::vector<uint8_t> hb;
		head.write(hb);
		memcpy(o, hb.data(), hb.size());
		auto put4 = [&](uint64_t at, uint32_t v) { for (int b = 0; b < 4; b++) o[at + b] = static_cast<uint8_t>((v >> (8 * b)) & 0xFF); };
		for (int64_t z = 0; z < sz; z++) put4(off_index + 4ull * z, cr.code_len[z]);
		put4(off_index + 4ull * sz, crc32c(o + off_index, 4ull * sz));
		if (!stored_model.empty()) memcpy(o + off_model, stored_model.data(), stored_model.size());
		for (int64_t z = 0; z < sz; z++) put4(off_tail + 4 + 4ull * z, fr.crcs[z]);
		put4(off_tail, labels_crc);
		e.device_stream_bytes = 0;
		if (e.keep_device_stream) {
			e.d_stream_out.ensure(total + 16);
			uint8_t* ds = e.d_stream_out.p;
			const void* up = head.label_format == FLAT ? o : nullptr;
			upload_small(ds, o, off_labels, s, up);
			if (label_bytes) {
				if (head.label_format == FLAT) copy_bytes_device(e.d_labels_bin.p, ds + off_labels, label_bytes, s);
				else CKL_HIP(hipMemcpyAsync(ds + off_labels, o + off_labels, label_bytes, hipMemcpyHostToDevice, s));
			}
			if (!stored_model.empty()) upload_small(ds + off_model, o + off_model, stored_model.size(), s, up);
			if (cr.total) copy_bytes_device(e.d_codes_out.p, ds + off_codes, cr.total, s);
			upload_small(ds + off_tail, o + off_tail, 4ull * (sz + 1), s, up);
			if (labels_stay) {
				CKL_HIP(hipStreamWaitEvent(s, e.ev_labels_crc, 0));
				CKL_HIP(hipMemcpyAsync(ds + off_tail, e.d_labels_crc.p, 4, hipMemcpyDeviceToDevice, s));
			}
			e.device_stream_bytes = total;
		}
		if (cr.total && !e.defer_codes) {
			if (e.async_host_copy && e.keep_device_stream) {
				if (!e.stream_copy) CKL_HIP(hipStreamCreateWithFlags(&e.stream_copy, hipStreamNonBlocking));
				if (!e.ev_codes) CKL_HIP(hipEventCreateWithFlags(&e.ev_codes, hipEventDisableTiming));
				CKL_HIP(hipEventRecord(e.ev_codes, s));
				CKL_HIP(hipStreamWaitEvent(e.stream_copy, e.ev_codes, 0));
				CKL_HIP(hipMemcpyAsync(o + off_codes, e.d_codes_out.p, cr.total, hipMemcpyDeviceToHost, e.stream_copy));
				if (labels_stay) {
					CKL_HIP(hipMemcpyAsync(o + off_labels, e.d_labels_bin.p, label_bytes, hipMemcpyDeviceToHost, e.stream_copy));
					CKL_HIP(hipMemcpyAsync(o + off_tail, e.d_labels_crc.p, 4, hipMemcpyDeviceToHost, e.stream_copy));
				}
				e.host_copy_pending = true;
			}
			else CKL_HIP(hipMemcpyAsync(o + off_codes, e.d_codes_out.p, cr.total, hipMemcpyDeviceToHost, s));
		}
		ht.mark("assembly");
		CKL_HIP(hipEventRecord(e.ev1, s));
		CKL_HIP(hipStreamSynchronize(s));
		ht.mark("codes_d2h");
		CKL_HIP(hipGetLastError());
		CKL_HIP(hipEventElapsedTime(&e.pipeline_ms, e.ev0, e.ev1));
		CKL_HIP(hipEventElapsedTime(&e.dominant_ms, e.evd0, e.evd1));
	}
	catch (...) {
		drain_host_copy(e, true);
		host_out_free(o);
		throw;
	}
	if (e.label_src) e.host_marks = ht.marks;
	*out = o;
	*out_len = total;
}

void check_dims(int64_t sx, int64_t sy, int64_t sz, int dtype_bytes, int is_signed);
struct ErodeSpec { int connectivity; bool keep_border; };
void recompress(const uint8_t* buf, uint64_t n, int markov_order, int device, uint8_t** out, uint64_t* out_len, const ErodeSpec* erode = nullptr) {
	if (erode && erode->connectivity != 6 && erode->connectivity != 18 && erode->connectivity != 26)
		throw Error(CKL_ERR_ARG, "crackle_amd: erode: connectivity must be 6, 18 or 26. Got: " + std::to_string(erode->connectivity));
	if (n < Header::kBytesV0) throw Error(CKL_ERR_FORMAT, "crackle: Input too small to be a valid stream. Bytes: " + std::to_string(n));
	const Header head = Header::parse(buf, n);
	if (head.is_signed) throw Error(CKL_ERR_ARG, "Signed integer data types are not currently supported.");
	const uint64_t order = markov_order < 0 ? static_cast<uint64_t>(head.markov_model_order) : static_cast<uint64_t>(markov_order);
	if (order > 15) throw Error(CKL_ERR_ARG, "crackle_amd: markov_model_order must be in [0, 15]");
	const int64_t sx = head.sx, sy = head.sy, sz = head.sz;
	check_dims(sx, sy, sz, head.data_width, 0);
	if (head.voxels() == 0) {
		hand_out(header_bytes(stream_header(head.data_width, sx, sy, sz, VolumeStats(), false, head.fortran_order, order, nullptr)), OutAlloc::MALLOC, out, out_len);
		return;
	}
	select_device(device);
	const bool prof = getenv("CKL_PROFILE") != nullptr;
	auto t_prev = std::chrono::steady_clock::now();
	auto lap = [&]() {
		const auto now = std::chrono::steady_clock::now();
		const double ms = std::chrono::duration<double, std::milli>(now - t_prev).count();
		t_prev = now;
		return ms;
	};
	DecoderPtr dec;
	const int rc = open_decoder(buf, n, 0, -1, device, dec);
	if (rc != CKL_OK) throw Error(rc, ckl_last_error());
	ckl_decoder& d = *dec;
	enter(&d);
	decoder_run(d, { Goal::TABLES });
	CKL_HIP(hipStreamSynchronize(d.stream));
	const double ms_tables = lap();

	ckl_encoder* raw = nullptr;
	if (ckl_encoder_create(sx, sy, sz, head.data_width, device, &raw) != CKL_OK) throw Error(CKL_ERR_RUNTIME, ckl_last_error());
	const EncoderPtr enc(raw);
	ckl_encoder& e = *enc;
	enter(&e);
	hipStream_t s = e.stream;
	const uint32_t ns = d.nslices;
	const RunArrays ra = run_arrays(d);
	RunLabels src;
	src.g = run_geom(d);
	src.word_base = ra.word_base; src.rbase = ra.rbase; src.run_cc = ra.run_cc; src.nruns = ra.nruns;
	src.comp_off = d.d_comp_off.p; src.ncomp = d.d_ncomp_expect.p; src.label_map = d.d_label_map.p;
	e.row_words = d.row_words;
	e.plane_words = d.plane_words;
	e.d_planes.ensure(2 * e.plane_words * ns);
	e.d_count_vh.ensure(4 * static_cast<size_t>(ns));
	e.d_stats.ensure(2);
	CKL_HIP(hipMemsetAsync(e.d_count_vh.p, 0, 3 * static_cast<size_t>(ns) * sizeof(uint32_t), s));
	CKL_HIP(hipMemsetAsync(e.d_stats.p, 0, sizeof(unsigned long long), s));
	CKL_HIP(hipEventRecord(e.evd0, s));
	const dim3 word_grid(static_cast<uint32_t>((e.plane_words + kBlock - 1) / kBlock), ns);
	if (erode) {
		const size_t pw = e.plane_words * ns;
		e.d_erode_bits.ensure(4 * pw);
		d.d_run_label.ensure(d.rtot);
		uint32_t *plane_p = e.d_erode_bits.p, *plane_c = plane_p + pw, *plane_d = plane_c + pw, *keep = plane_d + pw;
		const ErodeArgs ea = { static_cast<uint32_t>(erode->connectivity), erode->keep_border ? 1u : 0u, ns };
		hipLaunchKernelGGL(k_erode_run_labels, dim3(std::min<uint32_t>((d.max_rcap + kBlock - 1) / kBlock + 1, 256), ns), dim3(kBlock), 0, s, src, d.d_run_label.p);
		hipLaunchKernelGGL(k_erode_terms, word_grid, dim3(kBlock), 0, s, src, d.d_run_label.p, ea, plane_p, plane_c, plane_d);
		hipLaunchKernelGGL(k_erode_keep, word_grid, dim3(kBlock), 0, s, src, d.d_run_label.p, ea, plane_p, plane_c, plane_d, keep, e.d_stats.p);
		hipLaunchKernelGGL(k_erode_planes, word_grid, dim3(kBlock), 0, s, src, d.d_run_label.p, keep, plane_v(e), plane_h(e, ns), e.d_count_vh.p, ns);
		CKL_HIP(hipEventRecord(e.evd1, s));
		src.keep = keep;
	}
	else {
		hipLaunchKernelGGL(k_label_planes_from_runs, word_grid, dim3(kBlock), 0, s, src, plane_v(e), plane_h(e, ns), e.d_count_vh.p, ns);
		CKL_HIP(hipEventRecord(e.evd1, s));
		hipLaunchKernelGGL(k_label_map_max, dim3(static_cast<uint32_t>(std::min<uint64_t>((d.total_comp + kBlock - 1) / kBlock + 1, 1024))), dim3(kBlock), 0, s,
			d.d_label_map.p, d.total_comp, e.d_stats.p);
	}
	const std::vector<uint32_t> c = download(e.d_count_vh.p, 3 * static_cast<size_t>(ns), s);
	const std::vector<unsigned long long> mx = download(e.d_stats.p, 1, s);
	float ms_kernel = 0.f;
	CKL_HIP(hipEventElapsedTime(&ms_kernel, e.evd0, e.evd1));
	e.count_v.assign(c.begin(), c.begin() + ns);
	e.count_h.assign(c.begin() + ns, c.begin() + 2 * static_cast<size_t>(ns));
	VolumeStats st;
	st.max_label = mx[0];
	for (uint32_t zi = 0; zi < ns; zi++) st.pairs += static_cast<uint64_t>(sx - 1) * sy - e.count_v[zi] + c[2 * static_cast<size_t>(ns) + zi];
	e.planes_stats = st;
	e.planes_deferred = false;
	e.label_src = &src;
	e.planes_for = &src;
	e.planes_dims[0] = sx; e.planes_dims[1] = sy; e.planes_dims[2] = sz;
	const double ms_planes = lap();
	try {
		with_label_type(head.data_width, [&](auto t) {
			encode_typed<typename decltype(t)::type>(e, nullptr, sx, sy, sz, false, head.fortran_order, order, false, true, 0, nullptr, out, out_len);
		});
	}
	catch (...) { e.label_src = nullptr; throw; }
	e.label_src = nullptr;
	if (prof) {
		double graph = 0, cracks = 0, labels = 0, assembly = 0;
		for (const auto& m : e.host_marks) {
			const std::string name = m.first;
			if (name == "planes" || name == "graph") graph += m.second;
			else if (name == "cracks") cracks += m.second;
			else if (name == "assembly" || name == "codes_d2h") assembly += m.second;
			else labels += m.second;
		}
		if (erode) fprintf(stderr, "[ckl erode host ms] tables=%.2f keep_planes=%.2f graph=%.2f cracks=%.2f labels=%.2f assembly=%.2f k_erode_device=%.3f\n",
			ms_tables, ms_planes, graph, cracks, labels, assembly, ms_kernel);
		else fprintf(stderr, "[ckl recompress host ms] tables=%.2f label_planes=%.2f graph=%.2f cracks=%.2f labels=%.2f assembly=%.2f k_label_planes_from_runs_device=%.3f\n",
			ms_tables, ms_planes, graph, cracks, labels, assembly, ms_kernel);
	}
}

void reencode_markov(const uint8_t* buf, uint64_t n, int markov_order, int device, uint8_t** out, uint64_t* out_len) {
	if (n < Header::kBytesV0) throw Error(CKL_ERR_FORMAT, "crackle: Input too small to be a valid stream. Bytes: " + std::to_string(n));
	Header head = Header::parse(buf, n);
	if (markov_order < 0 || markov_order > 13) throw Error(CKL_ERR_ARG, "crackle_amd: markov_model_order must be in [0, 13] on device");
	if (head.markov_model_order == markov_order) { hand_out(buf, n, OutAlloc::HOST_OUT, out, out_len); return; }
	const bool v0 = head.format_version == 0;
	const uint64_t sz = head.sz;
	const uint64_t tail_bytes = v0 ? 0 : 4 * (sz + 1);
	const uint64_t off_index = head.header_bytes();
	const uint64_t off_labels = off_index + head.grid_index_bytes();
	if (!head.layout_fits(n)) throw Error(CKL_ERR_RUNTIME, "crackle: get_crack_code_offsets: Unable to read past end of buffer.");
	const uint64_t old_codes = off_labels + head.num_label_bytes + head.markov_model_bytes();
	uint64_t old_tail = old_codes;
	for (uint64_t z = 0; z < sz; z++) old_tail += rd_le(buf + off_index + 4 * z, 4);
	if (old_tail > n || tail_bytes > n - old_tail) throw Error(CKL_ERR_RUNTIME, "crackle: get_crack_codes: Unable to read past end of buffer.");

	const bool prof = getenv("CKL_PROFILE") != nullptr;
	auto t_prev = std::chrono::steady_clock::now();
	auto lap = [&](const char* what) {
		if (!prof) return;
		const auto now = std::chrono::steady_clock::now();
		fprintf(stderr, "[ckl reencode host ms] %s=%.2f\n", what, std::chrono::duration<double, std::milli>(now - t_prev).count());
		t_prev = now;
	};
	struct DecoderGuard { ckl_decoder* d = nullptr; ~DecoderGuard() { if (d) ckl_decoder_destroy(d); } } dec;
	struct EncoderGuard { ckl_encoder* e = nullptr; ~EncoderGuard() { if (e) ckl_encoder_destroy(e); } } enc;
	if (ckl_decoder_create(buf, n, 0, -1, device, &dec.d) != CKL_OK) throw Error(CKL_ERR_RUNTIME, ckl_last_error());
	lap("decoder_create");
	CrackResult cr;
	std::vector<uint8_t> stored_model;
	head.markov_model_order = markov_order;
	if (head.voxels() > 0) {
		const uint32_t *cv = nullptr, *ch = nullptr;
		uint32_t row_words = 0;
		uint64_t plane_words = 0;
		if (ckl_decoder_crack_planes(dec.d, &cv, &ch, &row_words, &plane_words) != CKL_OK) throw Error(CKL_ERR_RUNTIME, ckl_last_error());
		lap("crack_planes");
		if (ckl_encoder_create(head.sx, head.sy, head.sz, 1, device, &enc.e) != CKL_OK) throw Error(CKL_ERR_RUNTIME, ckl_last_error());
		lap("encoder_create");
		ckl_encoder& e = *enc.e;
		hipStream_t s = e.stream;
		const uint32_t ns = head.sz;
		const bool permissible = head.crack_format == PERMISSIBLE;
		e.row_words = row_words;
		e.plane_words = plane_words;
		e.d_planes.ensure(2 * plane_words * ns);
		e.d_count_vh.ensure(4 * static_cast<size_t>(ns));
		CKL_HIP(hipMemsetAsync(e.d_count_vh.p, 0, 2 * static_cast<size_t>(ns) * sizeof(uint32_t), s));
		hipLaunchKernelGGL(k_planes_from_cracks, dim3(static_cast<uint32_t>((plane_words + kBlock - 1) / kBlock), ns), dim3(kBlock), 0, s,
			cv, ch, head.sx, head.sy, row_words, plane_words, permissible ? 1u : 0u,
			plane_v(e), plane_h(e, ns), e.d_count_vh.p, ns);
		std::vector<uint32_t> c = download(e.d_count_vh.p, 2 * static_cast<size_t>(ns), s);
		e.count_v.assign(c.begin(), c.begin() + ns);
		e.count_h.assign(c.begin() + ns, c.end());
		lap("planes");
		graph_pass(e, head.sx, head.sy, head.sz, graph_format(permissible));
		lap("graph");
		CrackRequest crq;
		crq.permissible = permissible;
		crq.markov_order = markov_order;
		cr = crack_pass(e, head.sx, head.sy, head.sz, crq);
		lap("cracks");
		if (markov_order > 0) stored_model = markov_model_to_stored(cr.model);
	}
	else cr.code_len.assign(sz, 0);

	const uint64_t off_model = off_labels + head.num_label_bytes;
	const uint64_t off_codes = off_model + stored_model.size();
	const uint64_t off_tail = off_codes + cr.total;
	const uint64_t total = off_tail + tail_bytes;
	uint8_t* o = static_cast<uint8_t*>(host_out_alloc(total));
	try {
		if (cr.total) CKL_HIP(hipMemcpyAsync(o + off_codes, enc.e->d_codes_out.p, cr.total, hipMemcpyDeviceToHost, enc.e->stream));
		std::vector<uint8_t> hb;
		head.write(hb);
		memcpy(o, hb.data(), hb.size());
		auto put4 = [&](uint64_t at, uint32_t v) { for (int b = 0; b < 4; b++) o[at + b] = static_cast<uint8_t>((v >> (8 * b)) & 0xFF); };
		for (uint64_t z = 0; z < sz; z++) put4(off_index + 4 * z, cr.code_len[z]);
		if (!v0) put4(off_index + 4 * sz, crc32c(o + off_index, 4 * sz));
		memcpy(o + off_labels, buf + off_labels, head.num_label_bytes);
		if (!stored_model.empty()) memcpy(o + off_model, stored_model.data(), stored_model.size());
		if (tail_bytes) memcpy(o + off_tail, buf + old_tail, tail_bytes);
		if (cr.total) CKL_HIP(hipStreamSynchronize(enc.e->stream));
		lap("assembly");
	}
	catch (...) { host_out_free(o); throw; }
	*out = o;
	*out_len = total;
}

void check_dims(int64_t sx, int64_t sy, int64_t sz, int dtype_bytes, int is_signed) {
	if (is_signed) throw Error(CKL_ERR_ARG, "Signed integer data types are not currently supported.");
	if (dtype_bytes != 1 && dtype_bytes != 2 && dtype_bytes != 4 && dtype_bytes != 8) throw Error(CKL_ERR_ARG, "crackle_amd: dtype width must be 1, 2, 4 or 8 bytes");
	if (sx < 0 || sy < 0 || sz < 0) throw Error(CKL_ERR_ARG, "crackle_amd: negative dimension");
	if (sx > 0x7FFFFFF0ll || sy > 0x7FFFFFF0ll || sz > 0x7FFFFFF0ll) throw Error(CKL_ERR_ARG, "crackle_amd: dimension too large");
	if (static_cast<uint64_t>(sx + 1) * static_cast<uint64_t>(sy + 1) >= (1ull << 30)) throw Error(CKL_ERR_ARG, "crackle_amd: slices of 2^30 or more crack vertices are not supported");
}

}

extern "C" {

int ckl_encoder_create(int64_t sx, int64_t sy, int64_t sz, int dtype_bytes, int device, ckl_encoder** out) {
	return guard([&] {
		if (!out) throw Error(CKL_ERR_ARG, "crackle_amd: null argument");
		check_dims(sx, sy, sz, dtype_bytes, 0);
		select_device(device);
		std::unique_ptr<ckl_encoder> e(new ckl_encoder());
		e->device = device;
		e->dtype_bytes = dtype_bytes;
		CKL_HIP(hipStreamCreateWithFlags(&e->stream, hipStreamNonBlocking));
		{
			int lo = 0, hi = 0;
			CKL_HIP(hipDeviceGetStreamPriorityRange(&lo, &hi));
			CKL_HIP(hipStreamCreateWithPriority(&e->stream2, hipStreamNonBlocking, hi));
		}
		CKL_HIP(hipEventCreate(&e->ev0));
		CKL_HIP(hipEventCreate(&e->ev1));
		CKL_HIP(hipEventCreate(&e->evd0));
		CKL_HIP(hipEventCreate(&e->evd1));
		CKL_HIP(hipEventCreateWithFlags(&e->ev_in, hipEventDisableTiming));
		CKL_HIP(hipEventCreateWithFlags(&e->ev_prezero, hipEventDisableTiming));
		*out = e.release();
	});
}

int ckl_encoder_run(
	ckl_encoder* e, const void* labels_device, int64_t sx, int64_t sy, int64_t sz,
	int allow_pins, int fortran_order, uint64_t markov_model_order,
	int optimize_pins, int auto_bgcolor, int64_t manual_bgcolor,
	const ckl_encode_overrides* overrides, uint8_t** out, uint64_t* out_len
) {
	return guard([&] {
		if (!e || !out || !out_len) throw Error(CKL_ERR_ARG, "crackle_amd: null argument");
		check_dims(sx, sy, sz, e->dtype_bytes, 0);
		if (markov_model_order > 15) throw Error(CKL_ERR_ARG, "crackle_amd: markov_model_order must be in [0, 15]");
		enter(e);
		drain_host_copy(*e);
		const auto t_run0 = std::chrono::steady_clock::now();
		with_label_type(e->dtype_bytes, [&](auto t) {
			encode_typed(*e, static_cast<const typename decltype(t)::type*>(labels_device), sx, sy, sz, allow_pins != 0, fortran_order != 0,
				markov_model_order, optimize_pins != 0, auto_bgcolor != 0, manual_bgcolor, overrides, out, out_len);
		});
		if (getenv("CKL_PROFILE")) {
			fprintf(stderr, "[ckl encoder_run ms] encode=%.2f\n", std::chrono::duration<double, std::milli>(std::chrono::steady_clock::now() - t_run0).count());
		}
	});
}

int ckl_reencode_markov(const uint8_t* buf, uint64_t n, int markov_model_order, int device, uint8_t** out, uint64_t* out_len) {
	return guard([&] {
		if (!buf || !out || !out_len) throw Error(CKL_ERR_ARG, "crackle_amd: null argument");
		select_device(device);
		reencode_markov(buf, n, markov_model_order, device, out, out_len);
	});
}

int ckl_recompress(const uint8_t* buf, uint64_t n, int markov_model_order, int device, uint8_t** out, uint64_t* out_len) {
	return guard([&] {
		if (!buf || !out || !out_len) throw Error(CKL_ERR_ARG, "crackle_amd: null argument");
		recompress(buf, n, markov_model_order, device, out, out_len);
	});
}

int ckl_erode(const uint8_t* buf, uint64_t n, int connectivity, int flags, int markov_model_order, int device, uint8_t** out, uint64_t* out_len) {
	return guard([&] {
		if (!buf || !out || !out_len) throw Error(CKL_ERR_ARG, "crackle_amd: null argument");
		if (flags & ~CKL_ERODE_KEEP_BORDER) throw Error(CKL_ERR_ARG, "crackle_amd: erode: unknown flags");
		const ErodeSpec spec = { connectivity, (flags & CKL_ERODE_KEEP_BORDER) != 0 };
		recompress(buf, n, markov_model_order, device, out, out_len, &spec);
	});
}

int ckl_encoder_defer_codes(ckl_encoder* e, int defer) {
	if (!e) { set_last_error("crackle_amd: null encoder"); return CKL_ERR_ARG; }
	e->defer_codes = defer != 0;
	return CKL_OK;
}

int ckl_encoder_async_host_copy(ckl_encoder* e, int on) {
	if (!e) { set_last_error("crackle_amd: null encoder"); return CKL_ERR_ARG; }
	e->async_host_copy = on != 0;
	return CKL_OK;
}

int ckl_encoder_host_wait(ckl_encoder* e) {
	return guard([&] {
		if (!e) throw Error(CKL_ERR_ARG, "crackle_amd: null encoder");
		if (e->host_copy_pending) select_device(e->device);
		drain_host_copy(*e);
	});
}

int ckl_encoder_keep_device_stream(ckl_encoder* e, int keep) {
	if (!e) { set_last_error("crackle_amd: null encoder"); return CKL_ERR_ARG; }
	e->keep_device_stream = keep != 0;
	return CKL_OK;
}

int ckl_encoder_device_stream(const ckl_encoder* e, const uint8_t** stream_device, uint64_t* n_bytes) {
	if (!e || !stream_device || !n_bytes) { set_last_error("crackle_amd: null argument"); return CKL_ERR_ARG; }
	if (!e->device_stream_bytes) { set_last_error("crackle_amd: no device-resident stream (ckl_encoder_keep_device_stream before the run)"); return CKL_ERR_ARG; }
	*stream_device = e->d_stream_out.p;
	*n_bytes = e->device_stream_bytes;
	return CKL_OK;
}

int ckl_encoder_codes_to_host(ckl_encoder* e, uint8_t* dst_host, uint64_t capacity, uint64_t* n_bytes) {
	return guard([&] {
		if (!e || !n_bytes) throw Error(CKL_ERR_ARG, "crackle_amd: null argument");
		*n_bytes = e->last_codes_total;
		if (e->last_codes_total == 0) return;
		if (!dst_host || capacity < e->last_codes_total) throw Error(CKL_ERR_ARG, "crackle_amd: code buffer too small: need " + std::to_string(e->last_codes_total) + " bytes");
		select_device(e->device);
		if (e->async_host_copy) {
			if (!e->stream_copy) CKL_HIP(hipStreamCreateWithFlags(&e->stream_copy, hipStreamNonBlocking));
			CKL_HIP(hipMemcpyAsync(dst_host, e->d_codes_out.p, e->last_codes_total, hipMemcpyDeviceToHost, e->stream_copy));
			e->host_copy_pending = true;
			return;
		}
		CKL_HIP(hipMemcpyAsync(dst_host, e->d_codes_out.p, e->last_codes_total, hipMemcpyDeviceToHost, e->stream));
		CKL_HIP(hipStreamSynchronize(e->stream));
	});
}

int ckl_encoder_stats(
	ckl_encoder* e, const void* labels_device, int64_t sx, int64_t sy, int64_t sz,
	uint64_t* max_label, uint64_t* pixel_pairs, uint64_t* first_voxel, uint64_t* last_voxel
) {
	return guard([&] {
		enter(e);
		check_dims(sx, sy, sz, e->dtype_bytes, 0);
		const uint64_t voxels = static_cast<uint64_t>(sx) * sy * sz;
		VolumeStats st;
		e->planes_for = nullptr;
		if (voxels > 0) {
			uint64_t f = 0, l = 0;
			const uint8_t* base = static_cast<const uint8_t*>(labels_device);
			struct Drain { hipStream_t s; ~Drain() { (void)hipStreamSynchronize(s); } } drain{ e->stream };
			CKL_HIP(hipMemcpyAsync(&f, base, e->dtype_bytes, hipMemcpyDeviceToHost, e->stream));
			CKL_HIP(hipMemcpyAsync(&l, base + (voxels - 1) * e->dtype_bytes, e->dtype_bytes, hipMemcpyDeviceToHost, e->stream));
			planes_pass_any(*e, labels_device, sx, sy, sz, &st);
			CKL_HIP(hipStreamSynchronize(e->stream));
			st.first = f; st.last = l;
			e->planes_for = labels_device;
			e->planes_stats = st;
			e->planes_dims[0] = sx; e->planes_dims[1] = sy; e->planes_dims[2] = sz;
		}
		if (max_label) *max_label = st.max_label;
		if (pixel_pairs) *pixel_pairs = st.pairs;
		if (first_voxel) *first_voxel = st.first;
		if (last_voxel) *last_voxel = st.last;
	});
}

int ckl_encoder_markov_stats(
	ckl_encoder* e, const void* labels_device, int64_t sx, int64_t sy, int64_t sz,
	int crack_format, uint64_t markov_model_order, uint32_t* hist
) {
	return guard([&] {
		if (!e || !hist) throw Error(CKL_ERR_ARG, "crackle_amd: null argument");
		check_dims(sx, sy, sz, e->dtype_bytes, 0);
		if (markov_model_order == 0 || markov_model_order > 13) throw Error(CKL_ERR_ARG, "crackle_amd: markov_model_order must be in [1, 13]");
		enter(e);
		const size_t rows = static_cast<size_t>(1) << (2 * markov_model_order);
		std::vector<uint32_t> h(rows * 4, 0);
		if (static_cast<uint64_t>(sx) * sy * sz > 0) {
			CrackRequest crq;
			crq.goal = CrackGoal::HISTOGRAM;
			crq.permissible = crack_format == PERMISSIBLE;
			crq.markov_order = static_cast<int>(markov_model_order);
			const bool cached = planes_cached(*e, labels_device, sx, sy, sz);
			if (!cached) planes_pass_any(*e, labels_device, sx, sy, sz, nullptr);
			e->trail_for = nullptr;
			graph_pass(*e, sx, sy, sz, graph_format(crq.permissible));
			h = crack_pass(*e, sx, sy, sz, crq).hist;
			if (cached) { e->trail_for = labels_device; e->trail_perm = crq.permissible; e->trail_order = crq.markov_order; }
		}
		memcpy(hist, h.data(), h.size() * sizeof(uint32_t));
	});
}

static uint32_t* encoder_components(ckl_encoder* e, const void* labels_device, int64_t sx, int64_t sy, int64_t sz, uint32_t id_base, uint32_t* cc_device, uint32_t* ncomp_host) {
	check_dims(sx, sy, sz, e->dtype_bytes, 0);
	enter(e);
	const uint64_t voxels = static_cast<uint64_t>(sx) * sy * sz;
	if (voxels == 0) return cc_device;
	FlatResult fr;
	if (!planes_cached(*e, labels_device, sx, sy, sz)) planes_pass_any(*e, labels_device, sx, sy, sz, nullptr);
	flat_enqueue(*e, labels_device, sx, sy, sz, true, false);
	with_label_type(e->dtype_bytes, [&](auto t) { flat_collect(*e, static_cast<const typename decltype(t)::type*>(labels_device), sx, sy, sz, fr); });
	if (fr.total + id_base > 0xFFFFFFFFull) throw Error(CKL_ERR_RUNTIME, "crackle_amd: too many components");
	hipStream_t s2 = e->stream2;
	if (!cc_device) { e->d_cc_volume.ensure(voxels); cc_device = e->d_cc_volume.p; }
	launch_paint_components(s2, plane_v(*e), e->row_words, e->plane_words, sx, sy, sz, e->d_word_base.p, e->d_rbase.p, e->d_run_cc.p, e->d_comp_off.p, id_base, cc_device);
	for (int64_t z = 0; z < sz; z++) ncomp_host[z] = fr.ncomp[z];
	return cc_device;
}

int ckl_encoder_components(
	ckl_encoder* e, const void* labels_device, int64_t sx, int64_t sy, int64_t sz,
	uint32_t id_base, uint32_t* cc_host, uint32_t* ncomp_host
) {
	return guard([&] {
		if (!e || !cc_host || !ncomp_host) throw Error(CKL_ERR_ARG, "crackle_amd: null argument");
		const uint32_t* cc = encoder_components(e, labels_device, sx, sy, sz, id_base, nullptr, ncomp_host);
		const uint64_t voxels = static_cast<uint64_t>(sx) * sy * sz;
		if (voxels) CKL_HIP(hipMemcpyAsync(cc_host, cc, voxels * sizeof(uint32_t), hipMemcpyDeviceToHost, e->stream2));
		CKL_HIP(hipStreamSynchronize(e->stream2));
	});
}

int ckl_encoder_components_device(
	ckl_encoder* e, const void* labels_device, int64_t sx, int64_t sy, int64_t sz,
	uint32_t id_base, uint32_t* cc_device, uint32_t* ncomp_host
) {
	return guard([&] {
		if (!e || !cc_device || !ncomp_host) throw Error(CKL_ERR_ARG, "crackle_amd: null argument");
		encoder_components(e, labels_device, sx, sy, sz, id_base, cc_device, ncomp_host);
		CKL_HIP(hipStreamSynchronize(e->stream2));
	});
}

int ckl_encoder_last_timing(const ckl_encoder* e, float* pipeline_ms, float* dominant_kernel_ms) {
	if (!e) { set_last_error("crackle_amd: null encoder"); return CKL_ERR_ARG; }
	if (pipeline_ms) *pipeline_ms = e->pipeline_ms;
	if (dominant_kernel_ms) *dominant_kernel_ms = e->dominant_ms;
	return CKL_OK;
}

int ckl_encoder_walk_paths(ckl_encoder* e, uint32_t* fast_slices, uint32_t* compiled_slices) {
	return guard([&] {
		if (!e) throw Error(CKL_ERR_ARG, "crackle_amd: null encoder");
		uint32_t fast = 0, plain = 0;
		const size_t ns = e->last_trail_slices;
		if (ns && e->t_counters.p) {
			select_device(e->device);
			std::vector<uint32_t> nev(ns);
			CKL_HIP(hipMemcpy(nev.data(), e->t_counters.p + 5 * ns, ns * sizeof(uint32_t), hipMemcpyDeviceToHost));
			for (uint32_t v : nev) { if (v & (kEvFormatAddr12 | kEvWalkWide)) fast++; else if (v) plain++; }
		}
		if (fast_slices) *fast_slices = fast;
		if (compiled_slices) *compiled_slices = plain;
	});
}

int ckl_encoder_walk_step_kinds(ckl_encoder* e, uint32_t* counts, uint32_t max_slices, uint32_t* n_slices) {
	return guard([&] {
		if (!e || !counts || !n_slices) throw Error(CKL_ERR_ARG, "crackle_amd: null argument");
		const size_t ns = e->last_trail_slices;
		*n_slices = static_cast<uint32_t>(ns);
		if (!ns || !e->t_counters.p || !e->t_events.p) { *n_slices = 0; return; }
		if (ns > max_slices) throw Error(CKL_ERR_ARG, "crackle_amd: counts holds fewer slices than the last run had");
		select_device(e->device);
		DevBuf<uint32_t> d_counts;
		d_counts.ensure(ns * 5);
		hipLaunchKernelGGL(k_trail_step_kinds, dim3(static_cast<uint32_t>(ns)), dim3(kBlock), 0, e->stream, e->t_events.p, e->t_ibase.p, e->t_counters.p + 5 * ns, d_counts.p);
		CKL_HIP(hipMemcpyAsync(counts, d_counts.p, ns * 5 * sizeof(uint32_t), hipMemcpyDeviceToHost, e->stream));
		CKL_HIP(hipStreamSynchronize(e->stream));
	});
}

void ckl_encoder_destroy(ckl_encoder* e) { delete e; }

int ckl_compress(
	const void* labels, int labels_mem, int dtype_bytes, int is_signed,
	int64_t sx, int64_t sy, int64_t sz,
	int allow_pins, int fortran_order, uint64_t markov_model_order,
	int optimize_pins, int auto_bgcolor, int64_t manual_bgcolor,
	int device, uint8_t** out, uint64_t* out_len
) {
	ckl_encoder* e = nullptr;
	try {
		check_dims(sx, sy, sz, dtype_bytes, is_signed);
		if (!out || !out_len) throw Error(CKL_ERR_ARG, "crackle_amd: null argument");
		if (static_cast<uint64_t>(sx) * sy * sz == 0) {
			hand_out(header_bytes(stream_header(dtype_bytes, sx, sy, sz, VolumeStats(), allow_pins != 0, fortran_order != 0, markov_model_order, nullptr)), OutAlloc::MALLOC, out, out_len);
			return CKL_OK;
		}
	}
	catch (const Error& err) { set_last_error(err.what()); return err.status; }
	const int rc = ckl_encoder_create(sx, sy, sz, dtype_bytes, device, &e);
	if (rc != CKL_OK) return rc;
	const EncoderPtr owner(e);
	return guard([&]() -> int {
		const uint64_t bytes = static_cast<uint64_t>(sx) * sy * sz * dtype_bytes;
		const void* dev_labels = labels;
		DevBuf<uint8_t> tmp;
		if (labels_mem == CKL_MEM_HOST && bytes) {
			if (!labels) throw Error(CKL_ERR_ARG, "crackle_amd: null labels");
			tmp.ensure(bytes);
			CKL_HIP(hipMemcpy(tmp.p, labels, bytes, hipMemcpyHostToDevice));
			dev_labels = tmp.p;
		}
		return ckl_encoder_run(e, dev_labels, sx, sy, sz, allow_pins, fortran_order, markov_model_order,
			optimize_pins, auto_bgcolor, manual_bgcolor, nullptr, out, out_len);
	});
}

}
```

crackle_amd/csrc/ckl_encoder.hpp:

```cpp
#pragma once

#include "ckl_common.hpp"

#include <chrono>
#include <utility>

struct VolumeStats { uint64_t max_label = 0, pairs = 0, first = 0, last = 0; };
namespace ckl { namespace dev { struct RunLabels; } }

struct ckl_encoder {
	template <typename T> using DevBuf = ckl::DevBuf<T>;

	int device = 0;
	hipStream_t stream = nullptr;
	hipStream_t stream2 = nullptr;
	hipEvent_t ev0 = nullptr, ev1 = nullptr, ev_in = nullptr;
	hipEvent_t evd0 = nullptr, evd1 = nullptr;
	hipEvent_t ev_prezero = nullptr;
	float pipeline_ms = 0.f, dominant_ms = 0.f;
	int dtype_bytes = 0;

	DevBuf<unsigned long long> d_stats;
	DevBuf<uint4> d_adjm;
	DevBuf<uint32_t> d_slice_err;
	DevBuf<uint64_t> d_cbase, d_sbase, d_kbase, d_pbase, d_bbase, d_out_off, d_comp_off;
	DevBuf<uint32_t> d_ccap, d_scap, d_kcap;
	DevBuf<uint8_t> d_crack_tables;
	DevBuf<uint8_t> d_cp, d_fcode, d_dcode, d_payload, d_boc, d_codes_out, d_model;
	DevBuf<uint32_t> d_code_report;
	uint64_t codes_capacity = 0;
	bool defer_codes = false;
	bool keep_device_stream = false;
	bool async_host_copy = false;
	bool host_copy_pending = false;
	hipStream_t stream_copy = nullptr;
	hipStream_t stream_tab = nullptr;
	hipEvent_t ev_codes = nullptr;
	void* tables_staging = nullptr;
	bool uploads_by_kernel = false;
	hipEvent_t ev_labels_crc = nullptr;
	DevBuf<uint32_t> d_labels_crc;
	DevBuf<uint8_t> d_stream_out;
	uint64_t device_stream_bytes = 0;
	uint64_t last_codes_total = 0;
	DevBuf<uint32_t> d_stack_node, d_stack_code;
	DevBuf<uint32_t> d_chain_node, d_chain_off, d_chain_clen, d_chain_order, d_chain_dst, d_chain_vstart;
	DevBuf<uint32_t> d_n_chains, d_n_raw, d_n_valid, d_payload_len, d_boc_len;
	DevBuf<uint32_t> d_hist;
	DevBuf<uint32_t> d_planes, d_count_vh;
	uint32_t row_words = 0;
	uint64_t plane_words = 0;
	std::vector<uint32_t> count_v, count_h;
	DevBuf<uint64_t> d_rbase;
	DevBuf<uint32_t> d_rcap, d_word_base, d_parent, d_run_start, d_run_cc, d_comp_pix, d_nruns, d_ncomp, d_idbits, d_blk_roots;
	DevBuf<uint16_t> d_run_local;
	DevBuf<uint32_t> d_G, d_crc_acc;
	DevBuf<uint32_t> d_flat_report;
	uint64_t g_table_pixels = 0;
	DevBuf<uint64_t> d_mapping, d_sorted, d_uniq, d_label_hash, d_label_list;
	DevBuf<uint32_t> d_cc_volume;
	DevBuf<uint32_t> d_pin_kept, d_pin_u32;
	DevBuf<uint8_t> d_pin_tables;
	DevBuf<uint64_t> d_pin_u64;
	DevBuf<uint32_t> d_slice_err2, d_n_uniq, d_uniq_blk;
	DevBuf<uint8_t> d_labels_bin;
	const void* planes_for = nullptr;
	const void* trail_for = nullptr;
	bool trail_perm = false;
	int trail_order = 0;
	const ckl::dev::RunLabels* label_src = nullptr;
	DevBuf<uint32_t> d_erode_bits;
	std::vector<std::pair<const char*, double>> host_marks;
	VolumeStats planes_stats;
	int64_t planes_dims[3] = { 0, 0, 0 };
	std::vector<uint64_t> h_rbase;
	std::vector<uint32_t> h_rcap;
	std::vector<uint64_t> h_comp_off;
	DevBuf<uint16_t> s_run_lid, s_seam_first, s_seam_last;
	DevBuf<uint32_t> s_sc_w, s_sc_first, s_strip_nruns, s_strip_nsc;
	DevBuf<uint64_t> d_label_slots;
	uint32_t flat_nstrips = 0, flat_strip_rows = 0, flat_strip_cap = 0, flat_resolve_cap = 0;
	int max_lds = 0;
	bool flat_strips = false;
	std::vector<uint32_t> count_special, count_corner;
	DevBuf<uint32_t> d_plane_partial, t_blk_special, t_blk_corner;
	DevBuf<unsigned long long> d_plane_partial_max, d_plane_out;
	uint32_t graph_blocks = 0;
	uint32_t tiles_x = 0, tiles_y = 0, mtx2 = 0;
	uint64_t adjm_stride = 0;
	bool graph_permissible = false;
	bool planes_deferred = false;
	bool trail_zeroed = false;
	DevBuf<uint64_t> t_nbase, t_cobase, t_ibase;
	DevBuf<uint32_t> t_ncap, t_cocap, t_icap, t_max_steps;
	size_t last_trail_slices = 0;
	DevBuf<uint32_t> t_counters;
	DevBuf<uint32_t> t_node_vertex, t_vert2node, t_corner_vertex;
	DevBuf<uint8_t> t_node_adj;
	DevBuf<uint32_t> t_dart_end, t_dart_len, t_dart_minv, t_dart_minpos, t_parent, t_start_bits, t_starts;
	DevBuf<uint4> t_dart_codes;
	DevBuf<uint8_t> t_dart_inline;
	DevBuf<unsigned long long> t_compmin;
	DevBuf<uint32_t> t_items, t_item_off, t_chain_item0, t_events, t_chain_ev0, t_ev_lnd, t_ev_item;

	~ckl_encoder() {
		if (ev0) (void)hipEventDestroy(ev0);
		if (ev1) (void)hipEventDestroy(ev1);
		if (evd0) (void)hipEventDestroy(evd0);
		if (evd1) (void)hipEventDestroy(evd1);
		if (ev_in) (void)hipEventDestroy(ev_in);
		if (ev_prezero) (void)hipEventDestroy(ev_prezero);
		if (stream) (void)hipStreamDestroy(stream);
		if (stream2) (void)hipStreamDestroy(stream2);
		if (stream_copy) { (void)hipStreamSynchronize(stream_copy); (void)hipStreamDestroy(stream_copy); }
		if (stream_tab) { (void)hipStreamSynchronize(stream_tab); (void)hipStreamDestroy(stream_tab); }
		if (ev_codes) (void)hipEventDestroy(ev_codes);
		if (tables_staging) ckl::host_out_free(tables_staging);
		if (ev_labels_crc) (void)hipEventDestroy(ev_labels_crc);
	}
};

namespace ckl {

template <typename T>
inline std::vector<T> download(const T* p, size_t n, hipStream_t s) {
	std::vector<T> h(n);
	if (n) CKL_HIP(hipMemcpyAsync(h.data(), p, n * sizeof(T), hipMemcpyDeviceToHost, s));
	CKL_HIP(hipStreamSynchronize(s));
	return h;
}

struct HostTimer {
	bool on;
	std::chrono::steady_clock::time_point t0;
	std::vector<std::pair<const char*, double>> marks;
	HostTimer() : on(getenv("CKL_PROFILE") != nullptr), t0(std::chrono::steady_clock::now()) {}
	void mark(const char* name) {
		if (!on) return;
		auto t1 = std::chrono::steady_clock::now();
		marks.emplace_back(name, std::chrono::duration<double, std::milli>(t1 - t0).count());
		t0 = t1;
	}
	~HostTimer();
};
inline thread_local HostTimer* g_ht = nullptr;
#define HT_MARK(name) do { if (g_ht) g_ht->mark(name); } while (0)
inline HostTimer::~HostTimer() {
		g_ht = nullptr;
		if (!on) return;
		fprintf(stderr, "[ckl encode host ms]");
		for (auto& m : marks) fprintf(stderr, " %s=%.2f", m.first, m.second);
		fprintf(stderr, "\n");
}

inline void enter(ckl_encoder* e) {
	if (!e) throw Error(CKL_ERR_ARG, "crackle_amd: null encoder");
	select_device(e->device);
	wait_for_default_stream(e->stream, e->ev_in);
	wait_for_default_stream(e->stream2, e->ev_in);
}

inline void drain_host_copy(ckl_encoder& e, bool quiet = false) {
	if (!e.host_copy_pending) return;
	if (quiet) (void)hipStreamSynchronize(e.stream_copy);
	else CKL_HIP(hipStreamSynchronize(e.stream_copy));
	e.host_copy_pending = false;
}

enum class OutAlloc { MALLOC, HOST_OUT };
inline void hand_out(const uint8_t* bytes, size_t n, OutAlloc how, uint8_t** out, uint64_t* out_len) {
	uint8_t* p = static_cast<uint8_t*>(how == OutAlloc::MALLOC ? malloc(n ? n : 1) : host_out_alloc(n ? n : 1));
	if (!p) throw Error(CKL_ERR_RUNTIME, "crackle_amd: out of host memory");
	if (n) memcpy(p, bytes, n);
	*out = p;
	*out_len = n;
}
inline void hand_out(const std::vector<uint8_t>& bin, OutAlloc how, uint8_t** out, uint64_t* out_len) { hand_out(bin.data(), bin.size(), how, out, out_len); }

template <typename LABEL>
std::vector<uint8_t> pins_section_plain(
	ckl_encoder& e, const LABEL* labels, const uint32_t* cc, const uint64_t* comp_label, int64_t sx, int64_t sy, int64_t sz, uint64_t N,
	const std::vector<uint32_t>& nc, int index_width, int stored_width, bool auto_bgcolor, int64_t manual_bgcolor);

}
```

crackle_amd/csrc/ckl_trail.hpp:

```cpp
#pragma once

#include "ckl_device.hpp"

namespace ckl {
namespace dev {

constexpr uint32_t kTrailTileShift = 5, kTrailTileDim = 32;
__device__ __forceinline__ uint32_t mt_index(uint32_t mx, uint32_t my, uint32_t mtx2) {
	return (((my >> 1) * mtx2 + (mx >> 1)) << 2) | ((my & 1u) << 1) | (mx & 1u);
}
struct MicroTile {
	uint4 lo, hi;
	uint32_t mx, my;
	__device__ __forceinline__ bool holds(uint32_t x, uint32_t y) const { return (x >> 3) == mx && (y >> 3) == my; }
	__device__ __forceinline__ uint32_t nib(uint32_t x, uint32_t y) const {
		const uint32_t r = y & 7u;
		const uint32_t a0 = (r & 1u) ? lo.y : lo.x, a1 = (r & 1u) ? lo.w : lo.z, a2 = (r & 1u) ? hi.y : hi.x, a3 = (r & 1u) ? hi.w : hi.z;
		const uint32_t b0 = (r & 2u) ? a1 : a0, b1 = (r & 2u) ? a3 : a2;
		return (((r & 4u) ? b1 : b0) >> ((x & 7u) * 4u)) & 15u;
	}
};

enum : uint32_t { TRAIL_ERR_CAPACITY = 1u };
constexpr uint32_t kDartNone = 0xFFFFFFFFu;
constexpr uint32_t kItemSeg = 0u << 30, kItemCtl = 1u << 30, kItemDead = 2u << 30, kItemMask = 3u << 30;

struct TrailArgs {
	const uint4* adjm;
	uint64_t adjm_stride;
	uint32_t mtx2;
	uint32_t tiles_x, tiles_y;
	const uint32_t* planeV;
	const uint32_t* planeH;
	uint32_t row_words;
	uint64_t plane_words;
	uint32_t sx, sy, inv;
	uint32_t sxe, sye;
	uint32_t nverts;
	uint32_t z0;
	const uint32_t* max_steps;
	uint32_t graph_blocks;
	const uint32_t* blk_special;
	const uint32_t* blk_corner;
	const uint64_t* nbase;
	const uint32_t* ncap;
	uint32_t* n_nodes;
	uint32_t* node_vertex;
	uint8_t* node_adj;
	uint32_t* vert2node;
	const uint64_t* cobase;
	const uint32_t* cocap;
	uint32_t* n_corners;
	uint32_t* corner_vertex;
	uint32_t* dart_end;
	uint32_t* dart_len;
	uint32_t* dart_minv;
	uint32_t* dart_minpos;
	uint4* dart_codes;
	uint8_t* dart_inline;
	uint32_t* parent;
	unsigned long long* compmin;
	uint32_t* start_bits;
	uint32_t start_words;
	uint32_t* starts;
	uint32_t* n_starts;
	const uint64_t* ibase;
	const uint32_t* icap;
	uint32_t* items;
	uint32_t* item_off;
	uint32_t* n_items;
	const uint64_t* sbase;
	const uint32_t* scap;
	uint32_t* stack_node;
	uint32_t* stack_item;
	const uint64_t* kbase;
	const uint32_t* kcap;
	uint32_t* chain_node;
	uint32_t* chain_item0;
	uint32_t* chain_off;
	uint32_t* chain_clen;
	uint32_t* n_chains;
	uint32_t* n_raw;
	uint32_t* n_valid;
	const uint64_t* cbase;
	const uint32_t* ccap;
	uint8_t* cp;
	uint32_t* slice_err;
	uint32_t* events;
	uint32_t* n_events;
	uint32_t* seg_len_sum;
	uint32_t* chain_ev0;
	uint32_t* ev_lnd;
	uint32_t* ev_item;
	uint32_t walk_plain;
	uint32_t walk_stack_cap;
	uint32_t walk_no_regs;
	unsigned long long* dbg;
};

__device__ __forceinline__ void mt_load(MicroTile& c, const uint4* adjm, uint32_t x, uint32_t y, uint32_t mtx2) {
	const uint4* p = adjm + static_cast<uint64_t>(mt_index(x >> 3, y >> 3, mtx2)) * 2u;
	c.lo = p[0]; c.hi = p[1];
	c.mx = x >> 3; c.my = y >> 3;
}
__device__ __forceinline__ void trail_step(uint32_t& x, uint32_t& y, uint32_t k) {
	if (k & 2u) y = (k & 1u) ? y - 1u : y + 1u;
	else x = (k & 1u) ? x - 1u : x + 1u;
}
__device__ __forceinline__ uint32_t trail_code(uint32_t k) { return (0x0231u >> (4u * k)) & 3u; }

struct TileRowBits { uint32_t R, L, D, U; };

__device__ __forceinline__ TileRowBits trail_row_bits(
	const uint32_t* __restrict__ pv, const uint32_t* __restrict__ ph, uint32_t row_words,
	uint32_t sx, uint32_t sy, uint32_t tx, uint32_t y, uint32_t inv
) {
	const uint32_t x0 = tx << 5;
	const uint32_t lt_sx = x0 >= sx ? 0u : (sx - x0 >= 32u ? 0xFFFFFFFFu : ((1u << (sx - x0)) - 1u));
	const uint32_t le_sx = x0 > sx ? 0u : (sx - x0 >= 31u ? 0xFFFFFFFFu : ((2u << (sx - x0)) - 1u));
	const uint32_t ge_1 = tx == 0 ? 0xFFFFFFFEu : 0xFFFFFFFFu;
	TileRowBits b = { 0, 0, 0, 0 };
	const bool have_w = tx < row_words;
	if (y >= 1 && y < sy) {
		const uint32_t h = have_w ? ph[static_cast<uint64_t>(y) * row_words + tx] : 0u;
		const uint32_t hp = tx > 0 ? ph[static_cast<uint64_t>(y) * row_words + tx - 1] : 0u;
		b.R = (h ^ inv) & lt_sx;
		b.L = (((h << 1) | (hp >> 31)) ^ inv) & ge_1 & le_sx;
	}
	if (y < sy) b.D = ((have_w ? pv[static_cast<uint64_t>(y) * row_words + tx] : 0u) ^ inv) & ge_1 & lt_sx;
	if (y >= 1 && y <= sy) b.U = ((have_w ? pv[static_cast<uint64_t>(y - 1) * row_words + tx] : 0u) ^ inv) & ge_1 & lt_sx;
	return b;
}
__device__ __forceinline__ uint32_t trail_special_mask(const TileRowBits& b) {
	const uint32_t a1 = b.R ^ b.L, a2 = b.R & b.L, c1 = b.D ^ b.U, c2 = b.D & b.U;
	const uint32_t bit0 = a1 ^ c1, carry = a1 & c1;
	const uint32_t bit1 = a2 ^ c2 ^ carry, bit2 = (a2 & c2) | (carry & (a2 ^ c2));
	const uint32_t deg2 = ~bit0 & bit1 & ~bit2;
	return (b.R | b.L | b.D | b.U) & ~deg2;
}
__device__ __forceinline__ uint32_t trail_corner_mask(const TileRowBits& b) { return b.R & b.D & ~b.L & ~b.U; }
__device__ __forceinline__ uint32_t spread8(uint32_t m) {
	uint32_t x = (m | (m << 12)) & 0x000F000Fu;
	x = (x | (x << 6)) & 0x03030303u;
	x = (x | (x << 3)) & 0x11111111u;
	return x;
}

__device__ __forceinline__ void trail_rows8(
	const uint32_t* __restrict__ pv, const uint32_t* __restrict__ ph, uint32_t row_words,
	uint32_t sx, uint32_t sy, uint32_t tx, uint32_t y0, uint32_t inv, TileRowBits (&b)[8]
) {
#pragma unroll
	for (int k = 0; k < 8; k++) b[k] = TileRowBits{ 0, 0, 0, 0 };
	if (row_words == 0 || sy == 0) return;
	const uint32_t x0 = tx << 5;
	const uint32_t lt_sx = x0 >= sx ? 0u : (sx - x0 >= 32u ? 0xFFFFFFFFu : ((1u << (sx - x0)) - 1u));
	const uint32_t le_sx = x0 > sx ? 0u : (sx - x0 >= 31u ? 0xFFFFFFFFu : ((2u << (sx - x0)) - 1u));
	const uint32_t ge_1 = tx == 0 ? 0xFFFFFFFEu : 0xFFFFFFFFu;
	const bool have_w = tx < row_words;
	const uint32_t txc = have_w ? tx : row_words - 1u, txp = tx > 0 ? min(tx - 1u, row_words - 1u) : 0u;
	uint32_t hw[8], hpw[8], vw[9];
#pragma unroll
	for (uint32_t k = 0; k < 8; k++) {
		const uint64_t row = static_cast<uint64_t>(min(y0 + k, sy - 1u)) * row_words;
		hw[k] = ph[row + txc];
		hpw[k] = ph[row + txp];
	}
#pragma unroll
	for (uint32_t k = 0; k < 9; k++) {
		const uint32_t y = y0 + k;
		vw[k] = pv[static_cast<uint64_t>(min(y > 0 ? y - 1u : 0u, sy - 1u)) * row_words + txc];
	}
#pragma unroll
	for (uint32_t k = 0; k < 8; k++) {
		const uint32_t y = y0 + k;
		const uint32_t h = have_w ? hw[k] : 0u, hp = tx > 0 ? hpw[k] : 0u;
		if (y >= 1 && y < sy) {
			b[k].R = (h ^ inv) & lt_sx;
			b[k].L = (((h << 1) | (hp >> 31)) ^ inv) & ge_1 & le_sx;
		}
		if (y < sy) b[k].D = ((have_w ? vw[k + 1] : 0u) ^ inv) & ge_1 & lt_sx;
		if (y >= 1 && y <= sy) b[k].U = ((have_w ? vw[k] : 0u) ^ inv) & ge_1 & lt_sx;
	}
}

static __global__ void __launch_bounds__(kBlock) k_trail_graph(
	const uint32_t* __restrict__ planeV, const uint32_t* __restrict__ planeH, uint32_t row_words, uint64_t plane_words,
	uint32_t sx, uint32_t sy, uint32_t perm_mode, const unsigned long long* __restrict__ total_pairs, unsigned long long half_voxels,
	uint32_t* __restrict__ adjm_words, uint64_t adjm_stride_words,
	uint32_t mtx2, uint32_t tiles_x, uint32_t tiles_y, uint32_t* __restrict__ blk_special, uint32_t* __restrict__ blk_corner
) {
	__shared__ uint32_t s_red[2 * kWaves];
	__shared__ uint4 s_out[kWaves][kWave * 8];
	const int lane = threadIdx.x & 63, wave = threadIdx.x >> 6;
	const uint32_t zi = blockIdx.y;
	const bool permissible = perm_mode == 2u ? static_cast<long long>(*total_pairs) < static_cast<long long>(half_voxels) : perm_mode != 0u;
	const uint32_t item = blockIdx.x * kBlock + threadIdx.x;
	const uint32_t mtx = (sx + 1u + 7u) >> 3;
	uint32_t ns = 0, nc = 0;
	uint32_t my_base = 0, my_tiles = 0;
	if (item < tiles_x * tiles_y) {
		const uint32_t ty = item / tiles_x, tx = item - ty * tiles_x;
		TileRowBits b[8];
		trail_rows8(planeV + zi * plane_words, planeH + zi * plane_words, row_words, sx, sy, tx, ty << 3, permissible ? 0xFFFFFFFFu : 0u, b);
		my_base = mt_index(tx * 4u, ty, mtx2) * 32u;
		my_tiles = min(4u, mtx - min(mtx, tx * 4u));
#pragma unroll
		for (uint32_t q = 0; q < 4; q++) {
			uint32_t w[8];
#pragma unroll
			for (uint32_t k = 0; k < 8; k++)
				w[k] = spread8((b[k].R >> (8 * q)) & 255u) | (spread8((b[k].L >> (8 * q)) & 255u) << 1)
					| (spread8((b[k].D >> (8 * q)) & 255u) << 2) | (spread8((b[k].U >> (8 * q)) & 255u) << 3);
			s_out[wave][lane * 8 + ((2u * q) ^ (lane & 7))] = make_uint4(w[0], w[1], w[2], w[3]);
			s_out[wave][lane * 8 + ((2u * q + 1u) ^ (lane & 7))] = make_uint4(w[4], w[5], w[6], w[7]);
		}
#pragma unroll
		for (uint32_t k = 0; k < 8; k++) { ns += __popc(trail_special_mask(b[k])); nc += __popc(trail_corner_mask(b[k])); }
	}
	{
		uint8_t* dst = reinterpret_cast<uint8_t*>(adjm_words + zi * adjm_stride_words);
#pragma unroll
		for (uint32_t i = 0; i < 8; i++) {
			const uint32_t owner = i * 8u + (lane >> 3), p = lane & 7u;
			const uint32_t base = __shfl(my_base, owner, kWave), have = __shfl(my_tiles, owner, kWave);
			const uint4 v = s_out[wave][owner * 8u + (p ^ (owner & 7u))];
			const uint32_t q = p >> 1;
			if (q < have) *reinterpret_cast<uint4*>(dst + base + (q >> 1) * 128u + (q & 1u) * 32u + (p & 1u) * 16u) = v;
		}
	}
	ns = wave_sum(ns); nc = wave_sum(nc);
	if (lane == 0) { s_red[wave] = ns; s_red[kWaves + wave] = nc; }
	__syncthreads();
	if (threadIdx.x == 0) {
		uint32_t ts = 0, tc = 0;
		for (int w = 0; w < kWaves; w++) { ts += s_red[w]; tc += s_red[kWaves + w]; }
		blk_special[static_cast<uint64_t>(zi) * gridDim.x + blockIdx.x] = ts;
		blk_corner[static_cast<uint64_t>(zi) * gridDim.x + blockIdx.x] = tc;
	}
}

static __global__ void __launch_bounds__(kBlock) k_trail_count_scan(
	uint32_t* __restrict__ blk_special, uint32_t* __restrict__ blk_corner, uint32_t nblk,
	uint32_t* __restrict__ tot_special, uint32_t* __restrict__ tot_corner
) {
	__shared__ uint32_t s_scan[2 * kWaves];
	const uint32_t zi = blockIdx.x;
	uint32_t* bs = blk_special + static_cast<uint64_t>(zi) * nblk;
	uint32_t* bc = blk_corner + static_cast<uint64_t>(zi) * nblk;
	uint32_t cs = 0, cc = 0;
	for (uint32_t b0 = 0; b0 < nblk; b0 += kBlock) {
		const uint32_t b = b0 + threadIdx.x;
		uint32_t v[2] = { b < nblk ? bs[b] : 0u, b < nblk ? bc[b] : 0u }, tot[2];
		block_excl_add<2>(v, tot, s_scan);
		if (b < nblk) { bs[b] = cs + v[0]; bc[b] = cc + v[1]; }
		cs += tot[0]; cc += tot[1];
	}
	if (threadIdx.x == 0) { tot_special[zi] = cs; tot_corner[zi] = cc; }
}

static __global__ void __launch_bounds__(kBlock) k_trail_nodes(TrailArgs a) {
	__shared__ uint32_t s_scan[2 * kWaves];
	const uint32_t zi = blockIdx.y + a.z0;
	const uint32_t item = blockIdx.x * kBlock + threadIdx.x;
	TileRowBits b[8];
	uint32_t x0 = 0, y0 = 0;
	if (item < a.tiles_x * a.tiles_y) {
		const uint32_t ty = item / a.tiles_x, tx = item - ty * a.tiles_x;
		x0 = tx << kTrailTileShift; y0 = ty << 3;
		trail_rows8(a.planeV + zi * a.plane_words, a.planeH + zi * a.plane_words, a.row_words, a.sx, a.sy, tx, y0, a.inv, b);
	}
	else {
#pragma unroll
		for (int k = 0; k < 8; k++) b[k] = TileRowBits{ 0, 0, 0, 0 };
	}
	uint32_t v[2] = { 0, 0 }, tot[2];
#pragma unroll
	for (uint32_t k = 0; k < 8; k++) { v[0] += __popc(trail_special_mask(b[k])); v[1] += __popc(trail_corner_mask(b[k])); }
	block_excl_add<2>(v, tot, s_scan);
	uint32_t j = a.blk_special[static_cast<uint64_t>(zi) * a.graph_blocks + blockIdx.x] + v[0];
	uint32_t c = a.blk_corner[static_cast<uint64_t>(zi) * a.graph_blocks + blockIdx.x] + v[1];
	const uint64_t nb = a.nbase[zi];
	const uint32_t ncap = a.ncap[zi], cocap = a.cocap[zi];
	uint32_t err = 0;
#pragma unroll
	for (uint32_t k = 0; k < 8; k++) {
		const uint32_t y = y0 + k;
		const TileRowBits& r = b[k];
		for (uint32_t m = trail_special_mask(r); m; m &= m - 1u) {
			const uint32_t i = __ffs(m) - 1;
			const uint32_t vtx = y * a.sxe + x0 + i;
			if (j < ncap) {
				a.node_vertex[nb + j] = vtx;
				a.node_adj[nb + j] = static_cast<uint8_t>(((r.R >> i) & 1u) | (((r.L >> i) & 1u) << 1) | (((r.D >> i) & 1u) << 2) | (((r.U >> i) & 1u) << 3));
				a.vert2node[static_cast<uint64_t>(zi) * a.nverts + vtx] = j;
			}
			else err = TRAIL_ERR_CAPACITY;
			j++;
		}
		for (uint32_t m = trail_corner_mask(r); m; m &= m - 1u) {
			const uint32_t i = __ffs(m) - 1;
			if (c < cocap) a.corner_vertex[a.cobase[zi] + c] = y * a.sxe + x0 + i;
			else err = TRAIL_ERR_CAPACITY;
			c++;
		}
	}
	if (err) atomicOr(a.slice_err + zi, err);
	if (blockIdx.x == gridDim.x - 1 && threadIdx.x == kBlock - 1) {
		a.n_nodes[zi] = min(j, ncap);
		a.n_corners[zi] = min(c, cocap);
	}
}

constexpr uint32_t kWalkChunk = 192;
constexpr uint32_t kExpandChunk = 384;
constexpr int kWalkRefill = 8;
constexpr int kWalkAhead = 2;
constexpr uint32_t kInlineCodes = 64;

static __global__ void __launch_bounds__(kBlock) k_trail_segments(TrailArgs a) {
	__shared__ uint4 s_res[kWaves][kWalkChunk];
	__shared__ uint4 s_codes[kWaves][kWalkChunk];
	const uint32_t zi = blockIdx.y + a.z0;
	const uint32_t lane = threadIdx.x & (kWave - 1);
	const uint32_t wv = threadIdx.x >> 6;
	const uint32_t wave = blockIdx.x * kWaves + wv;
	const uint32_t n_darts = min(a.n_nodes[zi], a.ncap[zi]) * 4u;
	const uint32_t range_begin = wave * kWalkChunk;
	uint32_t next = range_begin;
	const uint32_t range_end = min(next + kWalkChunk, n_darts);
	if (next >= range_end) return;
	const uint64_t nb = a.nbase[zi];
	const uint4* adjm = a.adjm + zi * a.adjm_stride;
	const uint32_t* v2n = a.vert2node + static_cast<uint64_t>(zi) * a.nverts;
	const uint32_t cap = a.max_steps[zi];
	const unsigned long long lt_mask = (1ull << lane) - 1ull;
	uint4* res = s_res[wv];
	uint4* res_codes = s_codes[wv];
	for (uint32_t i = lane; i < kWalkChunk; i += kWave) res[i] = make_uint4(kDartNone, 0u, 0u, 0u);
	MicroTile c;
	c.lo = c.hi = make_uint4(0, 0, 0, 0); c.mx = c.my = 0xFFFFFFFFu;
	bool active = false;
	uint32_t d = 0, x = 0, y = 0, k = 0, steps = 0, minv = 0, minpos = 0, err = 0;
	uint4 cq = make_uint4(0, 0, 0, 0);
	auto push_code = [&](uint32_t kk) {
		cq.x = __builtin_amdgcn_alignbit(cq.y, cq.x, 2);
		cq.y = __builtin_amdgcn_alignbit(cq.z, cq.y, 2);
		cq.z = __builtin_amdgcn_alignbit(cq.w, cq.z, 2);
		cq.w = (cq.w >> 2) | (trail_code(kk) << 30);
	};
	unsigned long long dbg_iter = 0, dbg_lane = 0;
	const unsigned long long dbg_t0 = a.dbg ? __builtin_amdgcn_s_memtime() : 0ull;
	for (;;) {
		if (a.dbg) { dbg_iter++; dbg_lane += __popcll(__ballot(active)); }
		const unsigned long long need = __ballot(!active);
		const bool refill = next < range_end && (__popcll(need) >= kWalkRefill || need == ~0ull);
		const uint32_t cand = next + static_cast<uint32_t>(__popcll(need & lt_mask));
		const bool take = refill && !active && cand < range_end;
		uint32_t r_adj = 0, r_v0 = 0;
		if (take) { r_adj = a.node_adj[nb + (cand >> 2)]; r_v0 = a.node_vertex[nb + (cand >> 2)]; }
		if (active && !c.holds(x, y)) mt_load(c, adjm, x, y, a.mtx2);
		for (int it = 0; it < kWalkAhead; it++) {
			const bool go = active && c.holds(x, y);
			if (!__ballot(go)) break;
			if (go) {
				const uint32_t w = y * a.sxe + x;
				const uint32_t arr = k ^ 1u;
				if (w < minv) { minv = w; minpos = (steps << 2) | arr; }
				const uint32_t nib = c.nib(x, y);
				bool fin = false;
				if (__popc(nib) != 2) fin = true;
				else if (steps >= cap) { err = TRAIL_ERR_CAPACITY; fin = true; }
				else { k = __ffs(nib & ~(1u << arr)) - 1; push_code(k); trail_step(x, y, k); steps++; }
				if (fin) {
					res[d - range_begin] = make_uint4((w << 2) | arr, steps, minv, minpos);
					res_codes[d - range_begin] = cq;
					active = false;
				}
			}
		}
		if (take && ((r_adj >> (cand & 3u)) & 1u)) {
			d = cand; k = cand & 3u;
			y = r_v0 / a.sxe; x = r_v0 - y * a.sxe;
			minv = r_v0; minpos = 0;
			push_code(k);
			trail_step(x, y, k);
			steps = 1;
			active = true;
		}
		if (refill) next += static_cast<uint32_t>(__popcll(need));
		if (!__ballot(active) && next >= range_end) break;
	}
	if (a.dbg && lane == 0) {
		const unsigned long long cyc = __builtin_amdgcn_s_memtime() - dbg_t0;
		atomicAdd(a.dbg + 0, dbg_iter); atomicMax(a.dbg + 1, dbg_iter);
		atomicAdd(a.dbg + 2, cyc); atomicMax(a.dbg + 3, cyc);
		atomicAdd(a.dbg + 4, 1ull); atomicAdd(a.dbg + 5, dbg_lane);
	}
	const uint64_t db = nb * 4u + range_begin;
	uint32_t len_sum = 0;
	for (uint32_t i = lane; i < range_end - range_begin; i += kWave) {
		const uint4 r = res[i];
		a.dart_end[db + i] = r.x == kDartNone ? kDartNone : ((v2n[r.x >> 2] << 2) | (r.x & 3u));
		a.dart_len[db + i] = r.y;
		a.dart_minv[db + i] = r.z;
		a.dart_minpos[db + i] = r.w;
		const uint4 q = res_codes[i];
		const bool whole = r.x != kDartNone && r.y >= 1u && r.y <= kInlineCodes;
		uint4 o = make_uint4(0, 0, 0, 0);
		if (whole) {
			const uint32_t sh = 128u - 2u * r.y, w = sh >> 5, b = sh & 31u;
			const uint32_t v[5] = { q.x, q.y, q.z, q.w, 0u };
			auto word = [&](uint32_t t) -> uint32_t { return t == 0 ? v[0] : t == 1 ? v[1] : t == 2 ? v[2] : t == 3 ? v[3] : 0u; };
			auto pick = [&](uint32_t t) -> uint32_t { return __builtin_amdgcn_alignbit(word(t + w + 1u), word(t + w), b); };
			o = make_uint4(pick(0), pick(1), pick(2), pick(3));
			(void)v;
		}
		a.dart_codes[db + i] = o;
		a.dart_inline[db + i] = whole ? 1u : 0u;
		len_sum += r.x == kDartNone ? 0u : r.y;
	}
	len_sum = wave_sum(len_sum);
	if (lane == 0 && len_sum) atomicAdd(a.seg_len_sum + zi, len_sum);
	if (err) atomicOr(a.slice_err + zi, err);
}

static __global__ void __launch_bounds__(kBlock) k_trail_loops(TrailArgs a) {
	const uint32_t zi = blockIdx.y + a.z0;
	if (a.seg_len_sum[zi] == 2u * (a.max_steps[zi] - 1u)) return;
	const uint32_t ci = blockIdx.x * kBlock + threadIdx.x;
	const uint32_t nc = min(a.n_corners[zi], a.cocap[zi]);
	const uint4* adjm = a.adjm + zi * a.adjm_stride;
	const uint32_t cap = a.max_steps[zi];
	bool active = ci < nc;
	const uint32_t v0 = active ? a.corner_vertex[a.cobase[zi] + ci] : 0u;
	uint32_t y = v0 / a.sxe, x = v0 - y * a.sxe;
	uint32_t k = 0, steps = 1;
	trail_step(x, y, k);
	bool loop = false;
	MicroTile c;
	c.lo = c.hi = make_uint4(0, 0, 0, 0); c.mx = c.my = 0xFFFFFFFFu;
	while (__ballot(active)) {
		if (active && !c.holds(x, y)) mt_load(c, adjm, x, y, a.mtx2);
		for (int it = 0; it < kWalkAhead; it++) {
			const bool go = active && c.holds(x, y);
			if (!__ballot(go)) break;
			if (go) {
				const uint32_t w = y * a.sxe + x;
				const uint32_t nib = c.nib(x, y);
				if (w == v0) { loop = true; active = false; }
				else if (w < v0 || __popc(nib) != 2 || steps >= cap) active = false;
				else { k = __ffs(nib & ~(1u << (k ^ 1u))) - 1; trail_step(x, y, k); steps++; }
			}
		}
	}
	if (!loop) return;
	const uint32_t j = atomicAdd(a.n_nodes + zi, 1u);
	if (j >= a.ncap[zi]) { atomicOr(a.slice_err + zi, TRAIL_ERR_CAPACITY); return; }
	const uint64_t nb = a.nbase[zi];
	a.node_vertex[nb + j] = v0;
	a.node_adj[nb + j] = 5u;
	a.vert2node[static_cast<uint64_t>(zi) * a.nverts + v0] = j;
	const uint64_t db = (nb + j) * 4u;
	for (uint32_t q = 0; q < 4; q++) { a.dart_end[db + q] = kDartNone; a.dart_len[db + q] = 0; a.dart_minv[db + q] = v0; a.dart_minpos[db + q] = 0; a.dart_inline[db + q] = 0; }
	a.dart_end[db + 0] = (j << 2) | 2u; a.dart_len[db + 0] = steps;
	a.dart_end[db + 2] = (j << 2) | 0u; a.dart_len[db + 2] = steps;
}

template <bool LDS>
__device__ __forceinline__ uint32_t tuf_load(uint32_t* L, uint32_t i) {
	if (LDS) return __hip_atomic_load(L + i, __ATOMIC_RELAXED, __HIP_MEMORY_SCOPE_WORKGROUP);
	return __hip_atomic_load(L + i, __ATOMIC_RELAXED, __HIP_MEMORY_SCOPE_AGENT);
}
template <bool LDS>
__device__ __forceinline__ uint32_t tuf_find(uint32_t* L, uint32_t a) {
	uint32_t p = tuf_load<LDS>(L, a);
	while (p != a) {
		const uint32_t gp = tuf_load<LDS>(L, p);
		if (gp != p) atomicMin(L + a, gp);
		a = p;
		p = gp;
	}
	return a;
}
template <bool LDS>
__device__ __forceinline__ void tuf_unite(uint32_t* L, uint32_t a, uint32_t b) {
	for (;;) {
		a = tuf_find<LDS>(L, a);
		b = tuf_find<LDS>(L, b);
		if (a == b) return;
		if (a > b) { const uint32_t t = a; a = b; b = t; }
		const uint32_t old = atomicMin(L + b, a);
		if (old == b) return;
		b = old;
	}
}

constexpr uint32_t kStartList = 2048;
constexpr int kCompBlock = 256;

template <bool LDS, bool CMLDS>
__device__ __forceinline__ void trail_components_slice(const TrailArgs& a, uint32_t zi, uint32_t* parent, unsigned long long* compmin, uint32_t nn, uint32_t* s_scan, uint32_t* s_nstart) {
	const uint64_t nb = a.nbase[zi];
	uint32_t* start_tmp = a.items + a.ibase[zi];
	unsigned long long dg_t = a.dbg ? __builtin_amdgcn_s_memtime() : 0ull;
	auto stamp = [&](int slot) { if (a.dbg && threadIdx.x == 0) { const unsigned long long now = __builtin_amdgcn_s_memtime(); atomicAdd(a.dbg + slot, now - dg_t); dg_t = now; } };
	const uint32_t* dart_end = a.dart_end + nb * 4u;
	auto cm_load = [&](uint32_t j) -> unsigned long long {
		if (CMLDS) return __hip_atomic_load(compmin + j, __ATOMIC_RELAXED, __HIP_MEMORY_SCOPE_WORKGROUP);
		return __hip_atomic_load(compmin + j, __ATOMIC_RELAXED, __HIP_MEMORY_SCOPE_AGENT);
	};
	for (uint32_t j = threadIdx.x; j < nn; j += kCompBlock) parent[j] = j;
	__syncthreads();
	if (!LDS) __threadfence();
	constexpr uint32_t kNodeBatch = 4;
	for (uint32_t j0 = threadIdx.x; j0 < nn; j0 += kCompBlock * kNodeBatch) {
		uint4 e4[kNodeBatch], m4[kNodeBatch];
#pragma unroll
		for (uint32_t k = 0; k < kNodeBatch; k++) {
			const uint32_t j = j0 + k * kCompBlock;
			e4[k] = make_uint4(kDartNone, kDartNone, kDartNone, kDartNone);
			m4[k] = make_uint4(0u, 0u, 0u, 0u);
			if (j < nn) {
				e4[k] = *reinterpret_cast<const uint4*>(dart_end + j * 4u);
				m4[k] = *reinterpret_cast<const uint4*>(a.dart_minv + nb * 4u + j * 4u);
			}
		}
#pragma unroll
		for (uint32_t k = 0; k < kNodeBatch; k++) {
			const uint32_t j = j0 + k * kCompBlock;
			if (j >= nn) continue;
			const uint32_t ee[4] = { e4[k].x, e4[k].y, e4[k].z, e4[k].w }, mm[4] = { m4[k].x, m4[k].y, m4[k].z, m4[k].w };
			unsigned long long val = ~0ull;
#pragma unroll
			for (uint32_t q = 0; q < 4u; q++) {
				if (ee[q] == kDartNone) continue;
				const unsigned long long v = (static_cast<unsigned long long>(mm[q]) << 32) | (j * 4u + q);
				val = v < val ? v : val;
			}
			compmin[j] = val;
#pragma unroll
			for (uint32_t q = 0; q < 4u; q++) {
				if (ee[q] == kDartNone) continue;
				const uint32_t j2 = ee[q] >> 2;
				if (j < j2 && j2 < nn) tuf_unite<LDS>(parent, j, j2);
			}
		}
	}
	__syncthreads();
	if (!LDS || !CMLDS) __threadfence();
	stamp(12);
	for (uint32_t j0 = 0; j0 < nn; j0 += kCompBlock) {
		const uint32_t j = j0 + threadIdx.x;
		uint32_t root = 0xFFFFFFFFu;
		unsigned long long val = ~0ull;
		if (j < nn) {
			val = cm_load(j);
			if (val != ~0ull) {
				root = tuf_find<LDS>(parent, j);
				if (root == j) root = 0xFFFFFFFFu;
			}
// ... 1116 lines not shown
```

Baseline: 160.8 billion.

## Report counts via pinned host memory and cut per-call host setup overhead

Kernels now write slice counts, plane outputs and code-length reports straight into a persistent pinned host buffer, replacing separate device-to-host downloads with a single stream sync. Staging buffers are reused across calls, env-var parsing and the max-LDS device query are cached on the encoder, and hipFuncSetAttribute calls are skipped when the value is unchanged. The device-resident output stream is built early, with a small kernel copying the header, model and tail ranges, so it avoids a full host re-upload. This adds host-mapped-memory writes from kernels and more state to keep consistent across calls.

Result: no change. 160.7 billion (-0.1%).

```diff
diff --git a/crackle_amd/csrc/ckl_encode.hip b/crackle_amd/csrc/ckl_encode.hip
--- a/crackle_amd/csrc/ckl_encode.hip
+++ b/crackle_amd/csrc/ckl_encode.hip
@@ -993,6 +993,22 @@
 	}
 }
 
+struct StreamRanges { uint64_t off[3], len[3]; };
+__global__ void __launch_bounds__(kBlock) k_stream_small(const uint8_t* __restrict__ src_host, uint8_t* __restrict__ dst, StreamRanges r, const uint32_t* __restrict__ labels_crc) {
+	const uint64_t i = (static_cast<uint64_t>(blockIdx.x) * kBlock + threadIdx.x) * 16u;
+	const uint64_t off = blockIdx.y == 0 ? r.off[0] : blockIdx.y == 1 ? r.off[1] : r.off[2];
+	const uint64_t len = blockIdx.y == 0 ? r.len[0] : blockIdx.y == 1 ? r.len[1] : r.len[2];
+	if (i >= len) return;
+	const uint8_t* s = src_host + off + i;
+	uint8_t* d = dst + off + i;
+	if (i + 16u <= len && ((reinterpret_cast<uintptr_t>(s) | reinterpret_cast<uintptr_t>(d)) & 15u) == 0) *reinterpret_cast<uint4*>(d) = *reinterpret_cast<const uint4*>(s);
+	else for (uint64_t k = 0; k < 16u && i + k < len; k++) d[k] = s[k];
+	if (labels_crc && blockIdx.y == 2 && i == 0) {
+		const uint32_t c = labels_crc[0];
+		for (uint64_t b = 0; b < 4u && b < len; b++) d[b] = static_cast<uint8_t>((c >> (8u * b)) & 0xFFu);
+	}
+}
+
 __global__ void __launch_bounds__(kBlock) k_trail_step_kinds(const uint32_t* __restrict__ events, const uint64_t* __restrict__ ibase, const uint32_t* __restrict__ n_events, uint32_t* __restrict__ counts) {
 	__shared__ uint32_t s_c[5];
 	const uint32_t zi = blockIdx.x;
@@ -1059,13 +1075,17 @@
 		if (!src.empty()) memcpy(image.data() + off, src.data(), src.size() * sizeof(T));
 		items.push_back({ &dst, off, src.size(), [](void* b, uint8_t* base, size_t n) { static_cast<DevBuf<T>*>(b)->borrow(reinterpret_cast<T*>(base), n); } });
 	}
-	void commit(DevBuf<uint8_t>& block, hipStream_t s, void** staging = nullptr) {
+	void commit(DevBuf<uint8_t>& block, hipStream_t s, void** staging = nullptr, size_t* staging_bytes = nullptr) {
 		if (image.empty()) return;
 		for (const Item& it : items) it.bind(it.buf, nullptr, 0);
 		block.ensure(image.size());
 		if (staging) {
-			if (*staging) host_out_free(*staging);
-			*staging = host_out_alloc(std::max<size_t>(image.size(), 64u << 10));
+			if (!*staging || !staging_bytes || *staging_bytes < image.size()) {
+				if (*staging) host_out_free(*staging);
+				const size_t bytes = std::max<size_t>(image.size(), 64u << 10);
+				*staging = host_out_alloc(bytes);
+				if (staging_bytes) *staging_bytes = bytes;
+			}
 			memcpy(*staging, image.data(), image.size());
 			upload_small(block.p, *staging, image.size(), s, *staging);
 		}
@@ -1073,6 +1093,60 @@
 		for (const Item& it : items) it.bind(it.buf, block.p + it.off, it.count);
 	}
 };
+
+struct ReportLayout { size_t special, corner, planes, code, words; };
+inline ReportLayout report_layout(uint32_t ns) {
+	ReportLayout l;
+	l.special = 0; l.corner = ns; l.planes = 2ull * ns; l.code = 10ull * ns;
+	l.words = l.code + ns + 3;
+	return l;
+}
+
+bool report_block(ckl_encoder& e, uint32_t ns) {
+	if (e.sw.report_copy) return false;
+	const size_t words = report_layout(ns).words;
+	if (!e.report || e.report_words < words) {
+		if (e.report) {
+			CKL_HIP(hipStreamSynchronize(e.stream));
+			host_out_free(e.report);
+			e.report = nullptr;
+		}
+		const size_t bytes = std::max<size_t>(64u << 10, words * sizeof(uint32_t));
+		e.report = static_cast<uint32_t*>(host_out_alloc(bytes));
+		e.report_words = bytes / sizeof(uint32_t);
+		e.report_pinned = host_out_is_pinned(e.report);
+	}
+	return e.report_pinned;
+}
+
+void set_dynamic_lds(int device, int slot, const void* kernel, size_t bytes) {
+	constexpr int kDevices = 64, kSlots = 2;
+	static std::mutex m;
+	static long last[kDevices][kSlots];
+	const bool tracked = device >= 0 && device < kDevices && slot >= 0 && slot < kSlots;
+	std::lock_guard<std::mutex> lock(m);
+	if (tracked && last[device][slot] == static_cast<long>(bytes) + 1) return;
+	CKL_HIP(hipFuncSetAttribute(kernel, hipFuncAttributeMaxDynamicSharedMemorySize, static_cast<int>(bytes)));
+	if (tracked) last[device][slot] = static_cast<long>(bytes) + 1;
+}
+
+int max_lds_of(ckl_encoder& e) {
+	if (!e.max_lds) CKL_HIP(hipDeviceGetAttribute(&e.max_lds, hipDeviceAttributeMaxSharedMemoryPerBlock, e.device));
+	return e.max_lds;
+}
+
+void trail_presize(ckl_encoder& e, int64_t sx, int64_t sy, uint32_t ns) {
+	const uint64_t nverts = static_cast<uint64_t>(sx + 1) * (sy + 1);
+	e.d_slice_err.ensure(ns);
+	e.d_n_chains.ensure(ns); e.d_n_raw.ensure(ns); e.d_n_valid.ensure(ns);
+	e.d_payload_len.ensure(ns); e.d_boc_len.ensure(ns);
+	e.t_counters.ensure(7 * static_cast<size_t>(ns));
+	e.t_vert2node.ensure(nverts * ns);
+	e.t_start_bits.ensure(static_cast<size_t>((nverts + 31) / 32) * ns);
+	e.d_out_off.ensure(ns);
+	e.d_code_report.ensure(static_cast<size_t>(ns) + 3);
+	(void)max_lds_of(e);
+}
 
 template <typename LABEL>
 VolumeStats volume_stats(ckl_encoder& e, const LABEL* labels, uint64_t voxels) {
@@ -1134,6 +1208,7 @@
 	CKL_HIP(hipMemsetAsync(e.t_start_bits.p, 0, static_cast<size_t>(start_words) * ns * sizeof(uint32_t), s));
 	CKL_HIP(hipEventRecord(e.ev_prezero, s));
 	e.trail_zeroed = true;
+	e.prezero_awaited = false;
 }
 
 template <typename LABEL>
@@ -1206,16 +1281,32 @@
 		on_device ? e.d_plane_out.p + 4ull * ns : nullptr, half_voxels,
 		reinterpret_cast<uint32_t*>(e.d_adjm.p), e.adjm_stride * 4,
 		e.mtx2, e.tiles_x, e.tiles_y, e.t_blk_special.p, e.t_blk_corner.p);
+	const bool mapped = report_block(e, ns);
 	hipLaunchKernelGGL(k_trail_count_scan, dim3(ns), dim3(kBlock), 0, s, e.t_blk_special.p, e.t_blk_corner.p, e.graph_blocks,
-		e.d_count_vh.p + 2 * static_cast<size_t>(ns), e.d_count_vh.p + 3 * static_cast<size_t>(ns));
+		e.d_count_vh.p + 2 * static_cast<size_t>(ns), e.d_count_vh.p + 3 * static_cast<size_t>(ns),
+		mapped ? e.report : nullptr, e.planes_deferred ? e.d_plane_out.p : nullptr);
+	trail_presize(e, sx, sy, ns);
+	if (e.trail_zeroed && !e.prezero_awaited) { CKL_HIP(hipStreamWaitEvent(s, e.ev_prezero, 0)); e.prezero_awaited = true; }
 	std::vector<unsigned long long> po;
-	if (e.planes_deferred) {
-		po.resize(4ull * ns);
-		CKL_HIP(hipMemcpyAsync(po.data(), e.d_plane_out.p, po.size() * sizeof(unsigned long long), hipMemcpyDeviceToHost, s));
-	}
-	std::vector<uint32_t> c = download(e.d_count_vh.p + 2 * static_cast<size_t>(ns), 2 * static_cast<size_t>(ns), s);
-	e.count_special.assign(c.begin(), c.begin() + ns);
-	e.count_corner.assign(c.begin() + ns, c.end());
+	if (mapped) {
+		const ReportLayout rl = report_layout(ns);
+		CKL_HIP(hipStreamSynchronize(s));
+		e.count_special.assign(e.report + rl.special, e.report + rl.special + ns);
+		e.count_corner.assign(e.report + rl.corner, e.report + rl.corner + ns);
+		if (e.planes_deferred) {
+			po.resize(4ull * ns);
+			memcpy(po.data(), e.report + rl.planes, po.size() * sizeof(unsigned long long));
+		}
+	}
+	else {
+		if (e.planes_deferred) {
+			po.resize(4ull * ns);
+			CKL_HIP(hipMemcpyAsync(po.data(), e.d_plane_out.p, po.size() * sizeof(unsigned long long), hipMemcpyDeviceToHost, s));
+		}
+		std::vector<uint32_t> c = download(e.d_count_vh.p + 2 * static_cast<size_t>(ns), 2 * static_cast<size_t>(ns), s);
+		e.count_special.assign(c.begin(), c.begin() + ns);
+		e.count_corner.assign(c.begin() + ns, c.end());
+	}
 	VolumeStats v;
 	if (!po.empty()) planes_collect(e, ns, &v, &po);
 	if (st && !po.empty()) *st = v;
@@ -1282,8 +1373,7 @@
 	ta.cbase = e.d_cbase.p; ta.ccap = e.d_ccap.p; ta.cp = e.d_cp.p; ta.slice_err = e.d_slice_err.p;
 	ta.events = e.t_events.p; ta.n_events = e.t_counters.p + 5 * ns; ta.seg_len_sum = e.t_counters.p + 6 * ns; ta.chain_ev0 = e.t_chain_ev0.p; ta.ev_lnd = e.t_ev_lnd.p; ta.ev_item = e.t_ev_item.p;
 	ta.dbg = nullptr;
-	{ const char* env = getenv("CKL_TRAIL_WALK"); ta.walk_plain = (env && !strcmp(env, "plain")) ? 1u : 0u; ta.walk_no_regs = (env && !strcmp(env, "lds")) ? 1u : 0u; }
-	{ const char* env = getenv("CKL_TRAIL_WALK_STACK"); ta.walk_stack_cap = env ? static_cast<uint32_t>(std::max(1, atoi(env))) : 0xFFFFFFFFu; }
+	ta.walk_plain = e.sw.walk_plain; ta.walk_no_regs = e.sw.walk_no_regs; ta.walk_stack_cap = e.sw.walk_stack_cap;
 	ta.graph_blocks = e.graph_blocks; ta.blk_special = e.t_blk_special.p; ta.blk_corner = e.t_blk_corner.p;
 	ta.z0 = 0;
 	return ta;
@@ -1324,10 +1414,12 @@
 	const bool reuse_trail = rq.reuse_trail;
 	if (rq.goal == CrackGoal::HISTOGRAM && (!markov_order || rq.model)) throw Error(CKL_ERR_RUNTIME, "crackle_amd: internal: a markov histogram needs an order and no model");
 	CrackResult result;
+	const bool report_mapped = report_block(e, ns);
 	e.d_slice_err.ensure(ns);
 	const bool prezeroed = e.trail_zeroed && !reuse_trail;
 	e.trail_zeroed = false;
-	if (prezeroed) CKL_HIP(hipStreamWaitEvent(s, e.ev_prezero, 0));
+	if (prezeroed && !e.prezero_awaited) CKL_HIP(hipStreamWaitEvent(s, e.ev_prezero, 0));
+	e.prezero_awaited = false;
 	if (!reuse_trail && !prezeroed) CKL_HIP(hipMemsetAsync(e.d_slice_err.p, 0, ns * sizeof(uint32_t), s));
 
 	std::vector<uint64_t> cbase(ns), sbase(ns), kbase(ns);
@@ -1366,6 +1458,7 @@
 	HT_MARK("c:caps");
 
 	UploadPacker tables;
+	tables.image.reserve(15 * (static_cast<size_t>(ns) * sizeof(uint64_t) + 256));
 	tables.add(e.d_cbase, cbase); tables.add(e.d_ccap, ccap);
 	tables.add(e.d_sbase, sbase); tables.add(e.d_scap, scap);
 	tables.add(e.d_kbase, kbase); tables.add(e.d_kcap, kcap);
@@ -1391,7 +1484,7 @@
 	tables.add(e.t_cobase, cobase); tables.add(e.t_cocap, cocap);
 	tables.add(e.t_ibase, ibase); tables.add(e.t_icap, icap);
 	tables.add(e.t_max_steps, max_steps);
-	tables.commit(e.d_crack_tables, s, e.uploads_by_kernel ? &e.tables_staging : nullptr);
+	tables.commit(e.d_crack_tables, s, e.uploads_by_kernel ? &e.tables_staging : nullptr, &e.tables_staging_bytes);
 	HT_MARK("c:tables");
 	e.d_payload.ensure(ptot + 8); e.d_boc.ensure(btot + 8);
 	e.codes_capacity = ptot + btot;
@@ -1416,20 +1509,19 @@
 
 		TrailArgs ta = trail_args(e, sx, sy, ns);
 		const FinishArgs fa = finish_args(e, sx, sy, markov_order);
-		if (kTuning && getenv("CKL_TRAIL_DIAG")) { d_tdbg.ensure(16); CKL_HIP(hipMemsetAsync(d_tdbg.p, 0, 128, s)); ta.dbg = d_tdbg.p; }
-		int max_lds = 0;
-		CKL_HIP(hipDeviceGetAttribute(&max_lds, hipDeviceAttributeMaxSharedMemoryPerBlock, e.device));
+		if (kTuning && e.sw.trail_diag) { d_tdbg.ensure(16); CKL_HIP(hipMemsetAsync(d_tdbg.p, 0, 128, s)); ta.dbg = d_tdbg.p; }
+		const int max_lds = max_lds_of(e);
 		const size_t budget = static_cast<size_t>(max_lds > 1024 ? max_lds - 1024 : 0);
 		const uint32_t dart_blocks = (4 * max_ncap + kWalkChunk * kWaves - 1) / (kWalkChunk * kWaves);
 		size_t clds = (static_cast<size_t>(max_special) + 1024) * 12;
-		if (const char* env = getenv("CKL_TRAIL_LDS")) clds = static_cast<size_t>(std::max(0, atoi(env)));
+		if (e.sw.trail_lds >= 0) clds = static_cast<size_t>(e.sw.trail_lds);
 		clds = (std::min(budget, std::max<size_t>(clds, 1024)) / 16) * 16;
-		CKL_HIP(hipFuncSetAttribute(reinterpret_cast<const void*>(&k_trail_components), hipFuncAttributeMaxDynamicSharedMemorySize, static_cast<int>(clds)));
+		set_dynamic_lds(e.device, 0, reinterpret_cast<const void*>(&k_trail_components), clds);
 		size_t lds = trail_walk_lds(max_special);
-		if (const char* env = getenv("CKL_TRAIL_LDS")) lds = static_cast<size_t>(std::max(0, atoi(env)));
+		if (e.sw.trail_lds >= 0) lds = static_cast<size_t>(e.sw.trail_lds);
 		lds = std::min(budget, std::max<size_t>(lds, 4096));
 		lds = (lds / 16) * 16;
-		CKL_HIP(hipFuncSetAttribute(reinterpret_cast<const void*>(&k_trail_walk), hipFuncAttributeMaxDynamicSharedMemorySize, static_cast<int>(lds)));
+		set_dynamic_lds(e.device, 1, reinterpret_cast<const void*>(&k_trail_walk), lds);
 		trail_lds_used = lds;
 		HT_MARK("c:setup");
 
@@ -1448,13 +1540,14 @@
 		hipLaunchKernelGGL(k_finish, dim3(ns), dim3(kFinishBlock), 0, s, fa);
 	}
 	HT_MARK("c:enqueue");
-	if (kTuning && getenv("CKL_TRAIL_DIAG")) trail_diag(e, ns, d_tdbg.p, max_special, trail_lds_used);
+	if (kTuning && e.sw.trail_diag) trail_diag(e, ns, d_tdbg.p, max_special, trail_lds_used);
 
 	auto enqueue_tail = [&]() {
 		e.d_out_off.ensure(ns);
 		e.d_code_report.ensure(static_cast<size_t>(ns) + 3);
 		e.d_codes_out.ensure(e.codes_capacity + 8);
-		hipLaunchKernelGGL(k_code_offsets, dim3(1), dim3(kBlock), 0, s, e.d_boc_len.p, e.d_payload_len.p, e.d_slice_err.p, ns, e.d_out_off.p, e.d_code_report.p);
+		hipLaunchKernelGGL(k_code_offsets, dim3(1), dim3(kBlock), 0, s, e.d_boc_len.p, e.d_payload_len.p, e.d_slice_err.p, ns, e.d_out_off.p,
+			report_mapped ? e.report + report_layout(ns).code : e.d_code_report.p);
 		hipLaunchKernelGGL(k_gather_codes, dim3(ns), dim3(kBlock), 0, s, e.d_boc.p, e.d_bbase.p, e.d_boc_len.p,
 			e.d_payload.p, e.d_pbase.p, e.d_payload_len.p, e.d_out_off.p, e.d_codes_out.p);
 	};
@@ -1481,7 +1574,13 @@
 		enqueue_tail();
 	}
 	HT_MARK("c:finish_enq");
-	const std::vector<uint32_t> report = download(e.d_code_report.p, static_cast<size_t>(ns) + 3, s);
+	std::vector<uint32_t> report;
+	if (report_mapped) {
+		CKL_HIP(hipStreamSynchronize(s));
+		const uint32_t* r = e.report + report_layout(ns).code;
+		report.assign(r, r + ns + 3);
+	}
+	else report = download(e.d_code_report.p, static_cast<size_t>(ns) + 3, s);
 	HT_MARK("c:finish_wait");
 	if (report[ns + 2]) check_walk_errors(e, ns);
 	result.code_len.assign(report.begin(), report.begin() + ns);
@@ -1871,8 +1970,7 @@
 	if (!labels_first) {
 		uint32_t max_special = 0;
 		for (uint32_t v : e.count_special) max_special = std::max(max_special, v);
-		int max_lds = 0;
-		CKL_HIP(hipDeviceGetAttribute(&max_lds, hipDeviceAttributeMaxSharedMemoryPerBlock, e.device));
+		const int max_lds = max_lds_of(e);
 		labels_at_walk = max_special < 5000 && 2 * trail_walk_lds(max_special) + kFlatResolveLds <= static_cast<size_t>(max_lds);
 		if (!labels_at_walk) flat_enqueue(e, labels, sx, sy, sz, need_runs, false);
 	}
@@ -1916,6 +2014,7 @@
 	const int component_width = byte_width(static_cast<uint64_t>(sx) * sy);
 	hipStream_t s2 = e.stream2;
 	bool labels_stay = false;
+	bool resident_early = false;
 	auto label_side = [&]() {
 		if (labels_at_walk) {
 			CKL_HIP(hipStreamWaitEvent(s2, e.evd0, 0));
@@ -1936,9 +2035,15 @@
 			HT_MARK("label_table");
 			labels_stay = e.async_host_copy && e.keep_device_stream && !e.defer_codes && label_bytes > 0;
 			early_cap = off_labels + label_bytes + model_bytes_est + est_code_bytes + 4ull * (sz + 1) + 64;
-			early.p = host_out_alloc(early_cap);
+			early.p = host_out_alloc(e.keep_device_stream ? std::max<uint64_t>(early_cap, 64u << 10) : early_cap);
 			HT_MARK("l:buffer");
 			uint8_t* eo = static_cast<uint8_t*>(early.p);
+			if (e.keep_device_stream) {
+				e.d_stream_out.ensure(early_cap + 16);
+				e.device_stream_bytes = 0;
+				if (label_bytes) copy_bytes_device(e.d_labels_bin.p, e.d_stream_out.p + off_labels, label_bytes, s2);
+				resident_early = true;
+			}
 			if (labels_stay) {
 				e.d_labels_crc.ensure(1 + kBlock);
 				if (!e.ev_labels_crc) CKL_HIP(hipEventCreateWithFlags(&e.ev_labels_crc, hipEventDisableTiming));
@@ -1989,7 +2094,21 @@
 		for (int64_t z = 0; z < sz; z++) put4(off_tail + 4 + 4ull * z, fr.crcs[z]);
 		put4(off_tail, labels_crc);
 		e.device_stream_bytes = 0;
-		if (e.keep_device_stream) {
+		if (e.keep_device_stream && resident_early && total <= early_cap && host_out_is_pinned(o)) {
+			uint8_t* ds = e.d_stream_out.p;
+			StreamRanges sr;
+			sr.off[0] = 0; sr.len[0] = off_labels;
+			sr.off[1] = off_model; sr.len[1] = stored_model.size();
+			sr.off[2] = off_tail; sr.len[2] = 4ull * (sz + 1);
+			const uint64_t longest = std::max(sr.len[0], std::max(sr.len[1], sr.len[2]));
+			if (labels_stay) CKL_HIP(hipStreamWaitEvent(s, e.ev_labels_crc, 0));
+			hipLaunchKernelGGL(k_stream_small, dim3(static_cast<uint32_t>((longest + 16u * kBlock - 1) / (16u * kBlock)), 3), dim3(kBlock), 0, s,
+				o, ds, sr, labels_stay ? e.d_labels_crc.p : nullptr);
+			if (cr.total) copy_bytes_device(e.d_codes_out.p, ds + off_codes, cr.total, s);
+			e.device_stream_bytes = total;
+		}
+		else if (e.keep_device_stream) {
+			if (resident_early && labels_stay) CKL_HIP(hipEventSynchronize(e.ev_labels_crc));
 			e.d_stream_out.ensure(total + 16);
 			uint8_t* ds = e.d_stream_out.p;
 			const void* up = head.label_format == FLAT ? o : nullptr;
@@ -2274,6 +2393,19 @@
 		CKL_HIP(hipEventCreate(&e->evd1));
 		CKL_HIP(hipEventCreateWithFlags(&e->ev_in, hipEventDisableTiming));
 		CKL_HIP(hipEventCreateWithFlags(&e->ev_prezero, hipEventDisableTiming));
+		{
+			ckl_encoder::Switches& sw = e->sw;
+			const char* env = getenv("CKL_ENC_REPORT");
+			sw.report_copy = env && !strcmp(env, "copy");
+			env = getenv("CKL_TRAIL_WALK");
+			sw.walk_plain = (env && !strcmp(env, "plain")) ? 1u : 0u;
+			sw.walk_no_regs = (env && !strcmp(env, "lds")) ? 1u : 0u;
+			env = getenv("CKL_TRAIL_WALK_STACK");
+			sw.walk_stack_cap = env ? static_cast<uint32_t>(std::max(1, atoi(env))) : 0xFFFFFFFFu;
+			env = getenv("CKL_TRAIL_LDS");
+			sw.trail_lds = env ? std::max(0, atoi(env)) : -1;
+			sw.trail_diag = getenv("CKL_TRAIL_DIAG") != nullptr;
+		}
 		*out = e.release();
 	});
 }
diff --git a/crackle_amd/csrc/ckl_encoder.hpp b/crackle_amd/csrc/ckl_encoder.hpp
--- a/crackle_amd/csrc/ckl_encoder.hpp
+++ b/crackle_amd/csrc/ckl_encoder.hpp
@@ -37,7 +37,17 @@
 	hipStream_t stream_tab = nullptr;
 	hipEvent_t ev_codes = nullptr;
 	void* tables_staging = nullptr;
+	size_t tables_staging_bytes = 0;
 	bool uploads_by_kernel = false;
+	uint32_t* report = nullptr;
+	size_t report_words = 0;
+	bool report_pinned = false;
+	struct Switches {
+		bool report_copy = false;
+		uint32_t walk_plain = 0, walk_no_regs = 0, walk_stack_cap = 0xFFFFFFFFu;
+		long trail_lds = -1;
+		bool trail_diag = false;
+	} sw;
 	hipEvent_t ev_labels_crc = nullptr;
 	DevBuf<uint32_t> d_labels_crc;
 	DevBuf<uint8_t> d_stream_out;
@@ -91,6 +101,7 @@
 	bool graph_permissible = false;
 	bool planes_deferred = false;
 	bool trail_zeroed = false;
+	bool prezero_awaited = false;
 	DevBuf<uint64_t> t_nbase, t_cobase, t_ibase;
 	DevBuf<uint32_t> t_ncap, t_cocap, t_icap, t_max_steps;
 	size_t last_trail_slices = 0;
@@ -110,12 +121,13 @@
 		if (evd1) (void)hipEventDestroy(evd1);
 		if (ev_in) (void)hipEventDestroy(ev_in);
 		if (ev_prezero) (void)hipEventDestroy(ev_prezero);
-		if (stream) (void)hipStreamDestroy(stream);
+		if (stream) { if (report) (void)hipStreamSynchronize(stream); (void)hipStreamDestroy(stream); }
 		if (stream2) (void)hipStreamDestroy(stream2);
 		if (stream_copy) { (void)hipStreamSynchronize(stream_copy); (void)hipStreamDestroy(stream_copy); }
 		if (stream_tab) { (void)hipStreamSynchronize(stream_tab); (void)hipStreamDestroy(stream_tab); }
 		if (ev_codes) (void)hipEventDestroy(ev_codes);
 		if (tables_staging) ckl::host_out_free(tables_staging);
+		if (report) ckl::host_out_free(report);
 		if (ev_labels_crc) (void)hipEventDestroy(ev_labels_crc);
 	}
 };
diff --git a/crackle_amd/csrc/ckl_trail.hpp b/crackle_amd/csrc/ckl_trail.hpp
--- a/crackle_amd/csrc/ckl_trail.hpp
+++ b/crackle_amd/csrc/ckl_trail.hpp
@@ -242,7 +242,8 @@
 
 static __global__ void __launch_bounds__(kBlock) k_trail_count_scan(
 	uint32_t* __restrict__ blk_special, uint32_t* __restrict__ blk_corner, uint32_t nblk,
-	uint32_t* __restrict__ tot_special, uint32_t* __restrict__ tot_corner
+	uint32_t* __restrict__ tot_special, uint32_t* __restrict__ tot_corner,
+	uint32_t* __restrict__ host_report, const unsigned long long* __restrict__ plane_out
 ) {
 	__shared__ uint32_t s_scan[2 * kWaves];
 	const uint32_t zi = blockIdx.x;
@@ -257,6 +258,14 @@
 		cs += tot[0]; cc += tot[1];
 	}
 	if (threadIdx.x == 0) { tot_special[zi] = cs; tot_corner[zi] = cc; }
+	if (host_report) {
+		const uint32_t ns = gridDim.x;
+		if (threadIdx.x == 0) { host_report[zi] = cs; host_report[ns + zi] = cc; }
+		if (plane_out && threadIdx.x >= kWave && threadIdx.x < kWave + 4) {
+			const uint32_t k = threadIdx.x - kWave;
+			reinterpret_cast<unsigned long long*>(host_report + 2ull * ns)[4ull * zi + k] = plane_out[4ull * zi + k];
+		}
+	}
 }
 
 static __global__ void __launch_bounds__(kBlock) k_trail_nodes(TrailArgs a) {
```
